# ounben/fishnet

Hardware: AMD Instinct MI355X
Metric: NNUE evals/sec (node) at 1/2/4/8 MI355X + FT gather HBM GB/s as % of peak (higher is better)
Workload: dtype int16/int8

## Files before the change

fishnet_amd/build.py:

```python
from __future__ import annotations

import os
import subprocess
import sys

HERE = os.path.dirname(os.path.abspath(__file__))
ROOT = os.path.dirname(HERE)
CSRC = os.path.join(HERE, "csrc")
LIBDIR = os.path.join(HERE, "lib")
LIB = os.path.join(LIBDIR, "libgpu_nnue.so")
FAULT_LIB = os.path.join(LIBDIR, "libgpu_nnue_fault.so")
FAULT_DEFINES = ("-DGN_FAULT_PLAN_BLOCK=1",)
ODD_LIB = os.path.join(LIBDIR, "libgpu_nnue_d5.so")
ODD_DEFINES = ("-DGN_SMALL_DEPTH=5",)
SOURCES = ["gpu_nnue.hip", "kernels.hip", "stream.hip"]
HEADERS = ["chess.h", "host_board.h", "nnue.h", "kernels.h", "sha256.h", "device_util.h", "archive.h"]
ARCH = "gfx950"


def source_hash(defines=()) -> str:
    import hashlib
    h = hashlib.sha256()
    deps = [os.path.join(CSRC, f) for f in SOURCES + HEADERS] + [os.path.join(ROOT, "include", "gpu_nnue.h")]
    for d in deps:
        h.update(os.path.basename(d).encode() + b"\0")
        with open(d, "rb") as f:
            h.update(f.read())
    h.update(" ".join([ARCH, *defines]).encode())
    return h.hexdigest()


def _stale(lib: str, defines=()) -> bool:
    stamp = lib + ".sha256"
    if not os.path.exists(lib) or not os.path.exists(stamp):
        return True
    with open(stamp) as f:
        return f.read().strip() != source_hash(defines)


def build(force: bool = False, verbose: bool = False, defines=(), out: str | None = None) -> str:
    lib = out or LIB
    if not force and not _stale(lib, defines):
        return lib
    os.makedirs(LIBDIR, exist_ok=True)
    objs = []
    for src in SOURCES:
        obj = os.path.join(LIBDIR, src.replace(".hip", f".{os.getpid()}.o"))
        cmd = ["hipcc", f"--offload-arch={ARCH}", "-O3", "-std=c++17", "-fPIC", "-fvisibility=hidden",
               "-Wall", "-Wno-unused-function", *defines, "-c", os.path.join(CSRC, src), "-o", obj]
        if verbose:
            print(" ".join(cmd), flush=True)
        subprocess.run(cmd, check=True)
        objs.append(obj)
    tmp = lib + f".tmp{os.getpid()}"
    cmd = ["hipcc", f"--offload-arch={ARCH}", "-shared", "-fPIC", "-o", tmp] + objs + ["-lpthread"]
    subprocess.run(cmd, check=True)
    os.replace(tmp, lib)
    with open(lib + ".sha256", "w") as f:
        f.write(source_hash(defines) + "\n")
    for o in objs:
        os.remove(o)
    return lib


def build_rev(rev: str, out: str, defines=()) -> str:
    import shutil
    import tempfile
    tmp = tempfile.mkdtemp(prefix="gn_rev_")
    try:
        arch = subprocess.run(["git", "-C", ROOT, "archive", rev, "fishnet_amd/csrc", "include"],
                              check=True, capture_output=True).stdout
        subprocess.run(["tar", "-x", "-C", tmp], input=arch, check=True)
        objs = []
        for src in SOURCES:
            obj = os.path.join(tmp, src.replace(".hip", ".o"))
            subprocess.run(["hipcc", f"--offload-arch={ARCH}", "-O3", "-std=c++17", "-fPIC", "-fvisibility=hidden",
                            "-w", *defines, "-c", os.path.join(tmp, "fishnet_amd", "csrc", src), "-o", obj],
                           check=True)
            objs.append(obj)
        lib = os.path.join(LIBDIR, out)
        subprocess.run(["hipcc", f"--offload-arch={ARCH}", "-shared", "-fPIC", "-o", lib] + objs + ["-lpthread"],
                       check=True)
        return lib
    finally:
        shutil.rmtree(tmp, ignore_errors=True)


def build_fault(force: bool = False, verbose: bool = False) -> str:
    return build(force=force, verbose=verbose, defines=FAULT_DEFINES, out=FAULT_LIB)


def build_odd(force: bool = False, verbose: bool = False) -> str:
    return build(force=force, verbose=verbose, defines=ODD_DEFINES, out=ODD_LIB)


DROPIN_NATIVE = os.path.join(LIBDIR, "dropin_native")


def build_dropin_native(force: bool = False) -> str:
# ... 22 lines not shown
```

fishnet_amd/csrc/device_util.h:

```cpp
#pragma once
#include <hip/hip_runtime.h>

#include "nnue.h"

namespace gn {

typedef unsigned short ushort8 __attribute__((ext_vector_type(8)));
typedef int int4v __attribute__((ext_vector_type(4)));

__device__ __forceinline__ int32_t wmul(int32_t a, int32_t b) { return (int32_t)((uint32_t)a * (uint32_t)b); }
__device__ __forceinline__ int32_t wadd(int32_t a, int32_t b) { return (int32_t)((uint32_t)a + (uint32_t)b); }
__device__ __forceinline__ int clampi(int v, int lo, int hi) { return v < lo ? lo : v > hi ? hi : v; }
__device__ __forceinline__ uint32_t ft_row(uint32_t idx) { return idx < FT_INPUTS ? idx : FT_INPUTS - 1; }

__device__ __forceinline__ void load_tables(Tables &dst, const Tables *src) {
  const uint4 *s = reinterpret_cast<const uint4 *>(src);
  uint4 *d = reinterpret_cast<uint4 *>(&dst);
  for (int i = threadIdx.x; i < (int)(sizeof(Tables) / 16); i += blockDim.x) d[i] = s[i];
  __syncthreads();
}

template <bool U>
__device__ __forceinline__ int uni(int x) {
  if constexpr (U) return __builtin_amdgcn_readfirstlane(x);
  else return x;
}

__device__ __forceinline__ ushort8 ldft(const uint8_t *__restrict__ ft, uint32_t off) {
  return *reinterpret_cast<const ushort8 *>(ft + off);
}
__device__ __forceinline__ uint32_t ldpd(const uint8_t *__restrict__ ft, uint32_t off) {
  return *reinterpret_cast<const uint32_t *>(ft + off);
}
__device__ __forceinline__ int4v ldps(const uint8_t *__restrict__ ft, uint32_t off) {
  return *reinterpret_cast<const int4v *>(ft + off);
}

__device__ __forceinline__ int wave_features(const gn_board &p, uint16_t *rows_w, uint16_t *rows_b, int lane) {
  const uint64_t occ = p.occ;
  const int c = popcnt(occ);
  const bool has = (occ >> lane) & 1;
  const int k = popcnt(occ & ((1ull << lane) - 1));
  uint64_t wlo, whi;
  piece_words(p, wlo, whi);
  const int pc = has && k < 32 ? piece_nibble(wlo, whi, k) : 0;
  const int pt = pc & 7;
  const uint64_t bad = __ballot(has && (pt < PAWN || pt > KING));
  const uint64_t wkb = __ballot(has && pc == make_piece(WHITE, KING));
  const uint64_t bkb = __ballot(has && pc == make_piece(BLACK, KING));
  if (c < 2 || c > 32 || bad || popcnt(wkb) != 1 || popcnt(bkb) != 1) return 0;
  if (has) {
    if (rows_w) rows_w[k] = (uint16_t)feature_index(WHITE, lane, pc, __builtin_ctzll(wkb));
    if (rows_b) rows_b[k] = (uint16_t)feature_index(BLACK, lane, pc, __builtin_ctzll(bkb));
  }
  return c;
}

__device__ __forceinline__ int lane_piece(const gn_board &p, int lane) {
  const uint64_t occ = p.occ;
  const bool has = (occ >> lane) & 1;
  const int k = popcnt(occ & ((1ull << lane) - 1));
  uint64_t wlo, whi;
  piece_words(p, wlo, whi);
  return has && k < 32 ? piece_nibble(wlo, whi, k) : 0;
}

__device__ __forceinline__ int wave_features_excl(const gn_board &p, uint16_t *rows_w, uint16_t *rows_b, int lane,
                                                  uint64_t excl) {
  const uint64_t occ = p.occ;
  const int c = popcnt(occ);
  const bool has = (occ >> lane) & 1;
  const int pc = lane_piece(p, lane);
  const int pt = pc & 7;
  const uint64_t bad = __ballot(has && (pt < PAWN || pt > KING));
  const uint64_t wkb = __ballot(has && pc == make_piece(WHITE, KING));
  const uint64_t bkb = __ballot(has && pc == make_piece(BLACK, KING));
  if (c < 2 || c > 32 || bad || popcnt(wkb) != 1 || popcnt(bkb) != 1) return 0;
  if (has && !((excl >> lane) & 1)) {
    const int k = popcnt(occ & ~excl & ((1ull << lane) - 1));
    rows_w[k] = (uint16_t)feature_index(WHITE, lane, pc, __builtin_ctzll(wkb));
    rows_b[k] = (uint16_t)feature_index(BLACK, lane, pc, __builtin_ctzll(bkb));
  }
  return c;
}

__device__ __forceinline__ void wave_features_king_move(const gn_board &p, int h, int kfrom, int kto, int rfrom,
                                                        int rto, uint16_t *rows, int lane) {
  const uint64_t occ = p.occ;
  const bool has = (occ >> lane) & 1;
  const int k = popcnt(occ & ((1ull << lane) - 1));
  uint64_t wlo, whi;
  piece_words(p, wlo, whi);
  int pc = has && k < 32 ? piece_nibble(wlo, whi, k) : 0;
  if (lane == kfrom || lane == rfrom) pc = 0;
  if (lane == rto) pc = make_piece(h, ROOK);
  if (lane == kto) pc = make_piece(h, KING);
  const uint64_t cocc = __ballot(pc != 0);
  if (pc) rows[popcnt(cocc & ((1ull << lane) - 1))] = (uint16_t)feature_index(h, lane, pc, kto);
}

typedef short short2v __attribute__((ext_vector_type(2)));
typedef unsigned short ushort2v __attribute__((ext_vector_type(2)));
__device__ __forceinline__ uint2 transform8(ushort8 lo, ushort8 hi) {
  uint32_t o[4];
  const short2v z = {0, 0}, m = {254, 254};
#pragma unroll
  for (int i = 0; i < 4; ++i) {
    short2v a = {(short)lo[2 * i], (short)lo[2 * i + 1]}, b = {(short)hi[2 * i], (short)hi[2 * i + 1]};
    a = __builtin_elementwise_min(__builtin_elementwise_max(a, z), m);
    b = __builtin_elementwise_min(__builtin_elementwise_max(b, z), m);
    ushort2v pr = __builtin_bit_cast(ushort2v, a) * __builtin_bit_cast(ushort2v, b);
    pr = pr >> (ushort2v){9, 9};
    o[i] = __builtin_bit_cast(uint32_t, pr);
  }
  return make_uint2(__builtin_amdgcn_perm(o[1], o[0], 0x06040200u), __builtin_amdgcn_perm(o[3], o[2], 0x06040200u));
}

template <int L1, class Valid, class Emit>
__device__ __forceinline__ void layer_stack_wave(const NetDevice &net, const uint8_t *xt, uint8_t (*in1)[32],
                                                 int32_t *fwd, const int32_t (*psq)[2], int b, int lane,
                                                 Valid &&valid, Emit &&emit) {
  constexpr int XS = L1 + 16, KS = L1 / 64, BATCH = KS % 6 == 0 ? 6 : KS % 4 == 0 ? 4 : KS;
  static_assert(KS % BATCH == 0, "k-steps per batch");
  const int row = lane & 15, kg = lane >> 4;
  const int4v zero = {0, 0, 0, 0};
  const int4v wl = *reinterpret_cast<const int4v *>(net.w1 + ((size_t)b * 32 + row) * 32 + (kg & 1) * 16);
  const int4v wh = *reinterpret_cast<const int4v *>(net.w1 + ((size_t)b * 32 + 16 + row) * 32 + (kg & 1) * 16);
  const int32_t bias0 = net.b0[b * 16 + row];
  const int32_t b1l = net.b1[b * 32 + row], b1h = net.b1[b * 32 + 16 + row];
  const int32_t w2l = net.w2[b * 32 + row], w2h = net.w2[b * 32 + 16 + row];
  const int32_t b2v = net.b2[b];
  constexpr bool FRAG = L1 > 128;
  const int8_t *wb = FRAG ? net.w0f + ((size_t)b * KS * 64 + lane) * 16 : net.w0 + ((size_t)b * 16 + row) * L1 + kg * 16;
  const uint8_t *xa = xt + row * XS + kg * 16;
  int4v acc = zero;
#pragma unroll 1
  for (int k0 = 0; k0 < KS; k0 += BATCH) {
    int4v w[BATCH], a[BATCH];
#pragma unroll
    for (int j = 0; j < BATCH; ++j) w[j] = *reinterpret_cast<const int4v *>(wb + (FRAG ? 1024 : 64) * (k0 + j));
#pragma unroll
    for (int j = 0; j < BATCH; ++j) a[j] = *reinterpret_cast<const int4v *>(xa + 64 * (k0 + j));
#pragma unroll
    for (int j = 0; j < BATCH; ++j) acc = __builtin_amdgcn_mfma_i32_16x16x64_i8(a[j], w[j], acc, 0, 0, 0);
  }
#pragma unroll
  for (int i = 0; i < 4; ++i) {
    const int pos = 4 * kg + i;
    const int32_t v = wadd(acc[i], bias0);
    if (row < 15) {
      const long long s2 = ((long long)v * v) >> 19;
      in1[pos][row] = (uint8_t)(s2 < 127 ? s2 : 127);
      in1[pos][15 + row] = (uint8_t)clampi(v >> 6, 0, 127);
    } else {
      fwd[pos] = wmul(v, 600 * 16) / (127 * 64);
      in1[pos][30] = 0;
      in1[pos][31] = 0;
    }
  }
  __builtin_amdgcn_fence(__ATOMIC_RELEASE, "wavefront");
  __builtin_amdgcn_wave_barrier();
  __builtin_amdgcn_fence(__ATOMIC_ACQUIRE, "wavefront");
  const int4v a1 = kg < 2 ? *reinterpret_cast<const int4v *>(&in1[row][kg * 16]) : zero;
  const int4v cl = __builtin_amdgcn_mfma_i32_16x16x64_i8(a1, wl, zero, 0, 0, 0);
  const int4v ch = __builtin_amdgcn_mfma_i32_16x16x64_i8(a1, wh, zero, 0, 0, 0);
  int32_t part[4];
#pragma unroll
  for (int i = 0; i < 4; ++i) {
    const int32_t l = clampi(wadd(cl[i], b1l) >> 6, 0, 127), hh = clampi(wadd(ch[i], b1h) >> 6, 0, 127);
    part[i] = w2l * l + w2h * hh;
  }
#pragma unroll
  for (int off = 8; off; off >>= 1)
#pragma unroll
    for (int i = 0; i < 4; ++i) part[i] = wadd(part[i], __shfl_xor(part[i], off, 16));
  if (row == 0) {
#pragma unroll
    for (int i = 0; i < 4; ++i) {
      const int pos = 4 * kg + i;
      if (valid(pos, b)) {
        const int32_t positional = wadd(wadd(b2v, part[i]), fwd[pos]);
        const int32_t psqt = (int32_t)((uint32_t)psq[pos][0] - (uint32_t)psq[pos][1]) / 2;
        emit(pos, make_int2(psqt / 16, positional / 16));
      }
    }
  }
}

__device__ __forceinline__ int king_move_row(const gn_board &pb, int h, int kf, int kt, int rf, int rt, int lane,
                                             int &pos, int *piece = nullptr) {
  const uint64_t occ = pb.occ;
  const bool has = (occ >> lane) & 1;
  const int k = popcnt(occ & ((1ull << lane) - 1));
  uint64_t wlo, whi;
  piece_words(pb, wlo, whi);
  int pc = has && k < 32 ? piece_nibble(wlo, whi, k) : 0;
  if (lane == kf || lane == rf) pc = 0;
  if (lane == rt) pc = make_piece(h, ROOK);
  if (lane == kt) pc = make_piece(h, KING);
  const uint64_t cocc = __ballot(pc != 0);
  pos = popcnt(cocc & ((1ull << lane) - 1));
  if (piece) *piece = pc;
  return pc ? feature_index(h, lane, pc, kt) : -1;
}

__device__ __forceinline__ int king_move_row_pc(int pc, int h, int kf, int kt, int rf, int rt, int lane, int &pos,
                                                int &piece) {
  if (lane == kf || lane == rf) pc = 0;
  if (lane == rt) pc = make_piece(h, ROOK);
  if (lane == kt) pc = make_piece(h, KING);
  const uint64_t cocc = __ballot(pc != 0);
  pos = popcnt(cocc & ((1ull << lane) - 1));
  piece = pc;
  return pc ? feature_index(h, lane, pc, kt) : -1;
}

__device__ __forceinline__ int32_t wave_sum(int32_t v) {
#pragma unroll
  for (int off = 32; off; off >>= 1) v = wadd(v, __shfl_xor(v, off));
  return v;
}

template <class Op>
__device__ __forceinline__ uint32_t dpp_scan(uint32_t x, Op op) {
  x = op(x, (uint32_t)__builtin_amdgcn_update_dpp(0, (int)x, 0x111, 0xf, 0xf, true));
  x = op(x, (uint32_t)__builtin_amdgcn_update_dpp(0, (int)x, 0x112, 0xf, 0xf, true));
  x = op(x, (uint32_t)__builtin_amdgcn_update_dpp(0, (int)x, 0x114, 0xf, 0xf, true));
  x = op(x, (uint32_t)__builtin_amdgcn_update_dpp(0, (int)x, 0x118, 0xf, 0xf, true));
  x = op(x, (uint32_t)__builtin_amdgcn_update_dpp(0, (int)x, 0x142, 0xa, 0xf, false));
  x = op(x, (uint32_t)__builtin_amdgcn_update_dpp(0, (int)x, 0x143, 0xc, 0xf, false));
  return x;
}
__device__ __forceinline__ uint32_t scan_add(uint32_t x) {
  return dpp_scan(x, [](uint32_t a, uint32_t b) { return a + b; });
}
__device__ __forceinline__ uint32_t scan_or(uint32_t x) {
  return dpp_scan(x, [](uint32_t a, uint32_t b) { return a | b; });
}
__device__ __forceinline__ uint32_t or8(uint32_t x) {
  x |= (uint32_t)__builtin_amdgcn_update_dpp(0, (int)x, 0xb1, 0xf, 0xf, false);
  x |= (uint32_t)__builtin_amdgcn_update_dpp(0, (int)x, 0x4e, 0xf, 0xf, false);
  x |= (uint32_t)__builtin_amdgcn_update_dpp(0, (int)x, 0x141, 0xf, 0xf, false);
  return x;
}
__device__ __forceinline__ int32_t wave_sum_dpp(int32_t v) {
  return __builtin_amdgcn_readlane((int)scan_add((uint32_t)v), 63);
}

__device__ __forceinline__ void stage_fc1(int4v *w1s, const NetDevice &net) {
  for (int i = threadIdx.x; i < 8 * 32 * 2; i += blockDim.x) w1s[i] = reinterpret_cast<const int4v *>(net.w1)[i];
}
template <int NPART>
__device__ __forceinline__ void slice_sums(const int32_t *__restrict__ part, uint64_t npos, uint64_t q, int4v (&sums)[4]) {
#pragma unroll
  for (int r = 0; r < 4; ++r) {
    sums[r] = *reinterpret_cast<const int4v *>(part + q * 16 + 4 * r);
#pragma unroll
    for (int t = 1; t < NPART; ++t) {
      const int4v c = *reinterpret_cast<const int4v *>(part + ((uint64_t)t * npos + q) * 16 + 4 * r);
#pragma unroll
      for (int k = 0; k < 4; ++k) sums[r][k] = wadd(sums[r][k], c[k]);
    }
  }
}
__device__ __forceinline__ int2 slice_finish_from(const NetDevice &net, const int4v *w1s, const int4v (&sums)[4],
                                                  int2 info) {
  const int b = info.y & 7;
  int32_t v[16];
#pragma unroll
  for (int r = 0; r < 16; ++r) v[r] = wadd(sums[r >> 2][r & 3], net.b0[b * 16 + r]);
  uint32_t x[8] = {0, 0, 0, 0, 0, 0, 0, 0};
#pragma unroll
  for (int r = 0; r < 15; ++r) {
    const uint32_t u = v[r] < 0 ? 0u - (uint32_t)v[r] : (uint32_t)v[r], m = u < 8160u ? u : 8160u;
    const uint32_t a = (m * m) >> 19, c = (uint32_t)clampi(v[r] >> 6, 0, 127);
    x[r >> 2] |= a << (8 * (r & 3));
    x[(15 + r) >> 2] |= c << (8 * ((15 + r) & 3));
  }
  const int32_t fwd = wmul(v[15], 600 * 16) / (127 * 64);
  int32_t sum = 0;
#pragma unroll 4
  for (int o = 0; o < 32; ++o) {
    const int4v wa = w1s[(b * 32 + o) * 2], wb = w1s[(b * 32 + o) * 2 + 1];
    int32_t acc = 0;
#pragma unroll
    for (int d = 0; d < 4; ++d) acc = __builtin_amdgcn_sdot4((int)x[d], wa[d], acc, false);
#pragma unroll
    for (int d = 0; d < 4; ++d) acc = __builtin_amdgcn_sdot4((int)x[4 + d], wb[d], acc, false);
    const int32_t l = clampi(wadd(acc, net.b1[b * 32 + o]) >> 6, 0, 127);
    sum = wadd(sum, (int32_t)net.w2[b * 32 + o] * l);
  }
  const int32_t positional = wadd(wadd(net.b2[b], sum), fwd);
  return make_int2(info.x / 16, positional / 16);
}
template <int NPART>
__device__ __forceinline__ int2 slice_finish_one(const NetDevice &net, const int4v *w1s, const int32_t *__restrict__ part,
                                                 uint64_t npos, uint64_t q, int2 info) {
  int4v sums[4];
  slice_sums<NPART>(part, npos, q, sums);
  return slice_finish_from(net, w1s, sums, info);
}

}
```

fishnet_amd/csrc/gpu_nnue.hip:

```cpp
#include <stdarg.h>
#include <stdio.h>
#include <string.h>

#include <algorithm>
#include <atomic>
#include <chrono>
#include <condition_variable>
#include <memory>
#include <mutex>
#include <string>
#include <thread>
#include <vector>

#include "archive.h"
#include "host_board.h"
#include "kernels.h"
#include "sha256.h"

using namespace gn;

static thread_local std::string g_err;

static int fail(int code, const char *fmt, ...) {
  char buf[512];
// ... 159 lines not shown
  int mode = -1;
  uint64_t gen = 0;
  hipGraph_t graph = nullptr;
  hipGraphExec_t exec = nullptr;
  hipEvent_t done = nullptr;
  bool busy = false;
  gn_board *h_in = nullptr;
  gn_eval *h_out = nullptr;
  DevBuf<gn_board> all;
  DevBuf<gn_eval> rec;
  gn_board *in = nullptr, *r1 = nullptr, *r2 = nullptr;
  gn_eval *out = nullptr, *e1 = nullptr, *e2 = nullptr;
  DevBuf<uint64_t> off0, off1;
  DevBuf<uint16_t> m1, m2;
  DevBuf<int32_t> sv1, sv2;
  EvalBufs eb;
  ~FastBatch() {
    if (done) (void)hipEventDestroy(done);
    if (exec) (void)hipGraphExecDestroy(exec);
    if (graph) (void)hipGraphDestroy(graph);
    if (h_in) (void)hipHostFree(h_in);
    if (h_out) (void)hipHostFree(h_out);
    all.release(), rec.release();
    off0.release(), off1.release(), m1.release(), m2.release(), sv1.release(), sv2.release();
    eb.release();
  }
};

struct ExpSet {
  DevBuf<uint64_t> counts, offsets;
  DevBuf<uint32_t> owner;
  DevBuf<Board> unpacked;
  DevBuf<uint16_t> moves_tmp;
  const uint16_t *child_moves = nullptr;
  DevBuf<int2> pinfo;
  DevBuf<int2> p_osm, p_obg;
  DevBuf<uint8_t> p_nsm, p_nbg;
  EvalBufs eb;
  DevBuf<gn_board> children;
  int chain_k = 1;
  int slices = 1;
  bool planned = false;
  uint64_t etot = 0;
  void *scan_tmp = nullptr, *sort_tmp = nullptr;
  size_t scan_bytes = 0, sort_bytes = 0;
  hipEvent_t scored = nullptr;
  DevBuf<uint32_t> perr;
  DevBuf<unsigned long long> pstat;
  DevBuf<uint64_t> ent, eoff;
  DevBuf<TileDesc> tiles;
  DevBuf<uint32_t> btiles, border;
  void release() {
    perr.release(), pstat.release();
    ent.release(), eoff.release(), tiles.release(), btiles.release(), border.release();
    counts.release(), offsets.release(), owner.release(), unpacked.release(), moves_tmp.release();
    pinfo.release(), p_osm.release(), p_obg.release(), p_nsm.release(), p_nbg.release(), eb.release();
    children.release();
    if (scan_tmp) (void)hipFree(scan_tmp);
    if (sort_tmp) (void)hipFree(sort_tmp);
    scan_tmp = sort_tmp = nullptr, scan_bytes = sort_bytes = 0;
    if (scored) (void)hipEventDestroy(scored);
    scored = nullptr;
  }
};

struct Dev {
  int id = 0;
  hipStream_t stream = nullptr;
  void *net_mem[2] = {nullptr, nullptr};
  NetDevice net[2] = {};
  bool has[2] = {false, false};
  Tables *tables = nullptr;
  ExpSet cur, alt;
  DevBuf<gn_board> io_boards, frontier;
  DevBuf<gn_eval> io_out, io_out2;
  DevBuf<uint32_t> off32;
  DevBuf<uint16_t> moves;
  DevBuf<ChildDelta> deltas;
  DevBuf<uint64_t> kkeys, kkeys2;
  DevBuf<uint32_t> kidx, kperm;
  DevBuf<unsigned long long> sum;
  DevBuf<uint8_t> nslot;
  DevBuf<int32_t> part;
  bool part_locked = false;
  DevBuf<uint64_t> ebound;
  DevBuf<uint32_t> pool;
  DevBuf<uint16_t> bkeys, bkeys2;
  DevBuf<uint32_t> bidx;
  hipEvent_t done = nullptr;
  hipStream_t done_on = nullptr;
  float plan_ms = 0, stream_ms = 0, finish_ms = 0;
  struct ScoreLevel {
    DevBuf<uint64_t> sel, pos, counts, offsets;
    DevBuf<uint32_t> idx, owner;
    DevBuf<gn_board> boards, children;
    DevBuf<uint16_t> moves;
    DevBuf<gn_eval> ce;
    DevBuf<int32_t> sv;
    void release() {
      sel.release(), pos.release(), counts.release(), offsets.release(), idx.release(), owner.release();
      boards.release(), children.release(), moves.release(), ce.release(), sv.release();
    }
  } lv[2];
  hipStream_t copy = nullptr;
  hipEvent_t cev[2] = {nullptr, nullptr};
  DevBuf<gn_eval> po2[2], co2[2];
  DevBuf<gn_child> cc2[2];
  DevBuf<gn_line> ln2[2];
  hipEvent_t rev[2] = {nullptr, nullptr};
  DevBuf<uint16_t> mv2[2];
  DevBuf<gn_board> roots, rboards, par;
  DevBuf<uint64_t> moff;
  DevBuf<uint16_t> codes, smoves;
  DevBuf<int32_t> rstatus;
  DevBuf<uint32_t> gidx;
  double t_upload = 0, t_replay = 0, t_compute = 0, t_download = 0, t_tail = 0, t_rank = 0;
  std::unique_ptr<FastBatch> fast[6][3][2];
  std::condition_variable fast_cv;
  hipStream_t front = nullptr;
  hipEvent_t ev_streamed = nullptr, ev_planned = nullptr;
  std::mutex mu;
};

static void swap_sets(Dev &d) { std::swap(d.cur, d.alt); }

static hipError_t seq_begin(Dev &d, hipStream_t s) {
  if (d.done_on && d.done_on != s) return hipStreamWaitEvent(s, d.done, 0);
  return hipSuccess;
}
static hipError_t seq_end(Dev &d, hipStream_t s) {
  hipError_t e = hipEventRecord(d.done, s);
  if (e == hipSuccess) d.done_on = s;
  return e;
}
static int check_plan(Dev &d, hipStream_t s) {
  if (!d.cur.planned || !d.cur.perr.p) return GN_OK;
  uint32_t e = 0;
  HIP_TRY(hipMemcpyAsync(&e, d.cur.perr.p, sizeof(e), hipMemcpyDeviceToHost, s));
  HIP_TRY(hipStreamSynchronize(s));
  if (e) return fail(GN_E_HIP, "planned expansion failed on the device (error bits 0x%x)", e);
  return GN_OK;
}

struct SeqGuard {
  Dev &d;
  hipStream_t s;
  hipError_t e;
  bool ended = false;
  SeqGuard(Dev &d_, hipStream_t s_) : d(d_), s(s_) { e = seq_begin(d, s); }
  hipError_t finish() {
    ended = true;
    hipError_t r = seq_end(d, s);
    return r == hipSuccess ? hipStreamSynchronize(s) : r;
  }
  ~SeqGuard() {
    if (!ended) (void)seq_end(d, s);
  }
};

#ifndef GN_MAX_LEADERS
#define GN_MAX_LEADERS 1
#endif
constexpr int MAX_LEADERS = GN_MAX_LEADERS;
struct BatchReq {
  const gn_board *boards;
  size_t n;
// ... 23 lines not shown
  bool incremental = true;
  int swizzle = 9;
  int king_sort = 1;
  int chain = 81;
  bool king_cache = true;
  int stream_slices = 3;
  int64_t chunk_parents = 0;
  int l1[2] = {0, 0};
  uint32_t hash[2] = {0, 0};
  double t_parse = 0, t_total = 0;
};

enum { BIG = 0, SMALL = 1 };

static gn_eval_params default_params() {
  gn_eval_params P;
  P.small_net_threshold = 962;
  P.psqt_weight = 125;
  P.positional_weight = 131;
  P.reeval_threshold = 236;
  P.complexity_div_small = 18000;
  P.complexity_div_big = 18000;
  P.material_pawn_small = 535;
  P.material_pawn_big = 535;
  P.material_base = 77777;
  P.rule50_div = 212;
  P.value_clamp = 31506;
  const int32_t pv[5] = {208, 781, 825, 1276, 2538};
  memcpy(P.piece_value, pv, sizeof(pv));
  const double wa[4] = {-37.45051876, 121.19101539, -132.78783573, 420.70576692};
  memcpy(P.wdl_a, wa, sizeof(wa));
  P.wdl_material_min = 17;
  P.wdl_material_max = 78;
  P.wdl_material_anchor = 58;
  const int32_t ww[5] = {1, 3, 3, 5, 9};
  memcpy(P.wdl_piece_weight, ww, sizeof(ww));
  return P;
}

static size_t align256(size_t x) { return (x + 255) & ~(size_t)255; }

static int upload_net(Dev &d, int which, const HostNet &h) {
  const size_t RS = ft_row_stride((uint32_t)h.L1);
  size_t off[10], o = 0;
  const int carry = h.L1 == 128 ? 0 : CARRY_SLOTS;
  std::vector<int32_t> psqt((size_t)PSQT_BUCKETS * FT_ROWS);
  for (size_t r = 0; r < (size_t)FT_ROWS; ++r)
    for (int b = 0; b < PSQT_BUCKETS; ++b)
      memcpy(&psqt[(size_t)b * FT_ROWS + r], h.ft.data() + r * RS + 2 * (size_t)h.L1 + 4 * b, 4);
  const int KS = h.L1 / 64;
  std::vector<int8_t> w0f(h.w0.size());
  for (int b = 0; b < LAYER_STACKS; ++b)
    for (int ks = 0; ks < KS; ++ks)
      for (int ln = 0; ln < 64; ++ln)
        memcpy(&w0f[(((size_t)b * KS + ks) * 64 + ln) * 16],
               &h.w0[((size_t)b * 16 + (ln & 15)) * h.L1 + 64 * (size_t)ks + 16 * (ln >> 4)], 16);
  const size_t sz[10] = {((size_t)FT_ROWS + 4 * (size_t)carry + 128 * (size_t)carry + (carry ? 1 : 0)) * RS, h.bias.size() * 2, h.w0.size(), h.b0.size() * 4,
                         h.w1.size(), h.b1.size() * 4, h.w2.size(), h.b2.size() * 4, psqt.size() * 4, w0f.size()};
  const void *src[10] = {h.ft.data(), h.bias.data(), h.w0.data(), h.b0.data(),
                         h.w1.data(), h.b1.data(), h.w2.data(), h.b2.data(), psqt.data(), w0f.data()};
  for (int i = 0; i < 10; ++i) off[i] = o, o += align256(sz[i]);
  uint8_t *m = nullptr;
  if (hipMalloc(&m, o) != hipSuccess) return fail(GN_E_NOMEM, "device allocation of %zu bytes failed", o);
  d.net_mem[which] = m;
  for (int i = 0; i < 10; ++i)
    HIP_TRY(hipMemcpy(m + off[i], src[i], i == 0 ? (size_t)FT_ROWS * RS : sz[i], hipMemcpyHostToDevice));
  if (carry) HIP_TRY(hipMemset(m + off[0] + (size_t)FT_ROWS * RS, 0, 4 * (size_t)carry * RS));
  if (carry) HIP_TRY(hipMemset(m + off[0] + (size_t)ZERO_ROW * RS, 0, RS));
  NetDevice &n = d.net[which];
  n.L1 = h.L1;
  n.row_stride = (uint32_t)RS;
  n.carry_slots = carry;
  n.kc_slots = carry;
  n.ft = m + off[0];
  n.bias = reinterpret_cast<const int16_t *>(m + off[1]);
  n.w0 = reinterpret_cast<const int8_t *>(m + off[2]);
  n.b0 = reinterpret_cast<const int32_t *>(m + off[3]);
  n.w1 = reinterpret_cast<const int8_t *>(m + off[4]);
  n.b1 = reinterpret_cast<const int32_t *>(m + off[5]);
  n.w2 = reinterpret_cast<const int8_t *>(m + off[6]);
  n.b2 = reinterpret_cast<const int32_t *>(m + off[7]);
  n.psqt = reinterpret_cast<const int32_t *>(m + off[8]);
  n.w0f = reinterpret_cast<const int8_t *>(m + off[9]);
  d.has[which] = true;
  return GN_OK;
}

static void destroy(gn_ctx *ctx) {
  if (!ctx) return;
  for (auto &dp : ctx->devs) {
    Dev &d = *dp;
    (void)hipSetDevice(d.id);
    if (d.stream) (void)hipStreamSynchronize(d.stream);
    for (void *m : d.net_mem)
      if (m) (void)hipFree(m);
    if (d.tables) (void)hipFree(d.tables);
    d.cur.release(), d.alt.release();
    d.io_boards.release(), d.frontier.release(), d.io_out.release(), d.io_out2.release();
    d.off32.release(), d.moves.release(), d.sum.release(), d.deltas.release();
    d.part.release();
    if (d.front) (void)hipStreamSynchronize(d.front), (void)hipStreamDestroy(d.front);
    if (d.ev_streamed) (void)hipEventDestroy(d.ev_streamed);
    if (d.ev_planned) (void)hipEventDestroy(d.ev_planned);
    d.kkeys.release(), d.kkeys2.release(), d.kidx.release(), d.kperm.release();
    d.nslot.release();
    d.ebound.release(), d.pool.release();
    d.bkeys.release(), d.bkeys2.release(), d.bidx.release();
    d.lv[0].release(), d.lv[1].release();
    for (auto &row : d.fast)
      for (auto &pair : row)
        for (auto &f : pair) f.reset();
    for (int i = 0; i < 2; ++i) {
      d.po2[i].release(), d.co2[i].release(), d.cc2[i].release(), d.mv2[i].release(), d.ln2[i].release();
      if (d.rev[i]) (void)hipEventDestroy(d.rev[i]);
      if (d.cev[i]) (void)hipEventDestroy(d.cev[i]);
    }
    d.roots.release(), d.rboards.release(), d.par.release(), d.moff.release(), d.codes.release();
    d.smoves.release(), d.rstatus.release(), d.gidx.release();
    if (d.copy) (void)hipStreamSynchronize(d.copy), (void)hipStreamDestroy(d.copy);
    if (d.done) (void)hipEventDestroy(d.done);
    if (d.stream) (void)hipStreamDestroy(d.stream);
  }
  delete ctx;
}

static int create(const uint8_t *big, size_t big_len, const uint8_t *small, size_t small_len, const int *devices,
                  int n_devices, gn_ctx **out) {
  if (!out) return fail(GN_E_INVALID, "out is NULL");
  *out = nullptr;
  if (!big && !small) return fail(GN_E_INVALID, "no network given");
  HostNet hn[2];
  if (big) {
    int rc = parse_net(big, big_len, hn[BIG]);
    if (rc) return rc;
  }
  if (small) {
    int rc = parse_net(small, small_len, hn[SMALL]);
    if (rc) return rc;
  }
  int count = 0;
  if (hipGetDeviceCount(&count) != hipSuccess || count <= 0) return fail(GN_E_NODEVICE, "no HIP device visible");
  std::vector<int> ids;
  if (devices && n_devices > 0) ids.assign(devices, devices + n_devices);
  else ids.push_back(0);
  std::unique_ptr<gn_ctx, void (*)(gn_ctx *)> ctx(new gn_ctx(), destroy);
  ctx->P = default_params();
  for (int w = 0; w < 2; ++w) ctx->l1[w] = hn[w].L1, ctx->hash[w] = hn[w].hash;
  for (int id : ids) {
    if (id < 0 || id >= count) return fail(GN_E_NODEVICE, "device %d out of range (%d visible)", id, count);
    hipDeviceProp_t prop;
    HIP_TRY(hipGetDeviceProperties(&prop, id));
    if (!strstr(prop.gcnArchName, "gfx950"))
      return fail(GN_E_NODEVICE, "device %d is %s; libgpu_nnue is built for gfx950 only", id, prop.gcnArchName);
    ctx->devs.emplace_back(new Dev());
    Dev &d = *ctx->devs.back();
    d.id = id;
    HIP_TRY(hipSetDevice(id));
    HIP_TRY(hipStreamCreateWithFlags(&d.stream, hipStreamNonBlocking));
    HIP_TRY(hipEventCreateWithFlags(&d.done, hipEventDisableTiming));
    HIP_TRY(hipStreamCreateWithFlags(&d.copy, hipStreamNonBlocking));
#ifdef GN_AB_FRONT_PRIORITY
    {
      int least = 0, greatest = 0;
      HIP_TRY(hipDeviceGetStreamPriorityRange(&least, &greatest));
      HIP_TRY(hipStreamCreateWithPriority(&d.front, hipStreamNonBlocking, greatest));
    }
// ... 56 lines not shown
  DevBuf<int2> &osm = B.osm, &obg = B.obg;
  DevBuf<uint8_t> &nsm = B.nsm, &nbg = B.nbg;
  if (mode != GN_MODE_BIG) HIP_TRY(osm.ensure(n));
  if (mode != GN_MODE_SMALL) HIP_TRY(obg.ensure(n));
  if (mode == GN_MODE_FULL) {
    HIP_TRY(nsm.ensure(n));
    HIP_TRY(nbg.ensure(n));
  }
  auto mark = [&](int k) -> hipError_t { return ev ? hipEventRecord(ev[k], s) : hipSuccess; };
  const gn_eval_params &P = ctx->P;
  HIP_TRY(mark(0));
  const uint32_t *perm = nullptr;
  constexpr size_t KING_SORT_MIN = 1024;
  if (sort && (ctx->king_sort == 2 || (ctx->king_sort == 1 && n >= KING_SORT_MIN))) {
    if (n > 0x7FFFFFFFull) return fail(GN_E_INVALID, "king sort supports < 2^31 positions per call");
    HIP_TRY(d.kkeys.ensure(n));
    HIP_TRY(d.kkeys2.ensure(n));
    HIP_TRY(d.kidx.ensure(n));
    HIP_TRY(d.kperm.ensure(n));
    HIP_TRY(king_sort(b, n, d.kkeys.p, d.kidx.p, d.kkeys2.p, d.kperm.p, mode != GN_MODE_SMALL, d.cur.sort_tmp,
                      d.cur.sort_bytes, s));
    perm = d.kperm.p;
  }
  const int swz = (ctx->swizzle >> 1) & 1;
  HIP_TRY(mark(1));
  if (mode == GN_MODE_FULL && d.net[SMALL].L1 != 128) {
    HIP_TRY(launch_classify(b, n, P, nsm.p, nbg.p, s));
    HIP_TRY(launch_eval_net(d.net[SMALL], b, nsm.p, n, osm.p, perm, swz, s, nullptr));
    HIP_TRY(launch_reeval(osm.p, nsm.p, n, P, nbg.p, s));
  } else if (mode != GN_MODE_BIG)
    HIP_TRY(launch_eval_net(d.net[SMALL], b, nullptr, n, osm.p, perm, swz, s, mode == GN_MODE_SMALL ? rows_out : nullptr,
                            mode == GN_MODE_FULL ? &P : nullptr, nsm.p, nbg.p));
  HIP_TRY(mark(2));
  if (mode != GN_MODE_SMALL)
    HIP_TRY(launch_eval_net(d.net[BIG], b, mode == GN_MODE_FULL ? nbg.p : nullptr, n, obg.p, perm, swz, s,
                            rows_out));
  HIP_TRY(mark(3));
  HIP_TRY(launch_finalize(b, n, mode, osm.p, obg.p, nsm.p, nbg.p, P, d.tables, out, s, score, counts));
  HIP_TRY(mark(4));
  return GN_OK;
}

static Dev *slot(gn_ctx *ctx, int s) {
  if (!ctx || s < 0 || s >= (int)ctx->devs.size()) return nullptr;
  return ctx->devs[s].get();
}

template <class F>
static void parallel_for(size_t n, size_t grain, F &&f) {
  unsigned hw = std::max(1u, std::min(16u, std::thread::hardware_concurrency()));
  size_t chunks = std::min<size_t>(hw, (n + grain - 1) / std::max<size_t>(grain, 1));
  if (chunks <= 1) {
    f(0, n);
    return;
  }
  std::vector<std::thread> th;
  size_t per = (n + chunks - 1) / chunks;
  for (size_t c = 0; c < chunks; ++c) {
    size_t lo = c * per, hi = std::min(n, lo + per);
    if (lo < hi) th.emplace_back([=, &f] { f(lo, hi); });
  }
  for (auto &t : th) t.join();
}

static int chain_len(const gn_ctx *ctx, Dev &d, size_t n) {
  if (!ctx->incremental || (ctx->chain >= -1 && ctx->chain <= 1) || !d.has[BIG] || !d.net[BIG].carry_slots)
    return 1;
  if (ctx->chain < 0) return -ctx->chain;
  size_t k = (size_t)ctx->chain;
  if ((n + k - 1) / k < 2048) k = std::max<size_t>(2, std::min(k, n / 2048));
  return (int)k;
}

static bool plan_path(const gn_ctx *ctx, const Dev &d, int mode) {
  return mode != GN_MODE_SMALL && ctx->incremental && d.has[BIG] &&
         (d.net[BIG].L1 == 3072 || d.net[BIG].L1 == 1024);
}

static int finalize_all(gn_ctx *ctx, Dev &d, const gn_board *parents, const gn_board *children, int mode,
                        gn_eval *parent_out, gn_eval *child_out, size_t n, size_t total, hipStream_t s,
                        bool score_parents, bool sliced = false) {
  const gn_eval_params &P = ctx->P;
  const ExpSet &x = d.cur;
  const SlicedOut sc = {&d.net[BIG], d.part.p, x.pinfo.p, (uint64_t)(n + total), (uint64_t)n},
                  sp = {&d.net[BIG], d.part.p, x.pinfo.p, (uint64_t)(n + total), 0};
  const bool fast = x.child_moves != nullptr;
  HIP_TRY(launch_finalize(children, total, mode, x.eb.osm.p, x.eb.obg.p, x.eb.nsm.p, x.eb.nbg.p, P, d.tables, child_out,
                          s, 0, nullptr, fast ? x.owner.p : nullptr, fast ? x.child_moves : nullptr,
                          fast ? x.unpacked.p : nullptr, sliced ? &sc : nullptr));
  if (parent_out)
    HIP_TRY(launch_finalize(parents, n, mode, x.p_osm.p, x.p_obg.p, x.p_nsm.p, x.p_nbg.p, P, d.tables, parent_out, s,
                            score_parents ? 1 : 0, x.counts.p, nullptr, nullptr, nullptr, sliced ? &sp : nullptr));
  return GN_OK;
}

static hipError_t count_children(Dev &d, const gn_board *parents, size_t n, hipStream_t s, size_t *total) {
  ExpSet &x = d.cur;
  hipError_t e;
  if ((e = x.counts.ensure(n + 1)) != hipSuccess || (e = x.offsets.ensure(n + 1)) != hipSuccess) return e;
  if ((e = hipMemsetAsync(x.counts.p + n, 0, sizeof(uint64_t), s)) != hipSuccess) return e;
  if ((e = launch_count_children(parents, n, d.tables, x.counts.p, s)) != hipSuccess) return e;
  if ((e = exclusive_scan_u64(x.counts.p, x.offsets.p, n + 1, x.scan_tmp, x.scan_bytes, s)) != hipSuccess) return e;
  uint64_t t = 0;
  if ((e = hipMemcpyAsync(&t, x.offsets.p + n, sizeof(t), hipMemcpyDeviceToHost, s)) != hipSuccess) return e;
  if ((e = hipStreamSynchronize(s)) != hipSuccess) return e;
  *total = (size_t)t;
  return hipSuccess;
}

struct GenOpts {
  hipEvent_t *ev = nullptr;
  unsigned long long *rows = nullptr;
  bool deltas = false;
  int chain_k = 1;
  bool plan = false;
  bool skip_internal = false;
  bool trusted = false;
  size_t limit = SIZE_MAX;
};
static int generate_children(Dev &d, const gn_board *parents, size_t n, gn_board *children_or_null, uint16_t *moves,
                             size_t *total, hipStream_t s, const GenOpts &o = {}) {
  ExpSet &x = d.cur;
  x.chain_k = o.deltas ? o.chain_k : 1;
  x.planned = o.deltas && o.plan;
  if (x.planned) {
    HIP_TRY(hipMemsetAsync(x.perr.p, 0, sizeof(uint32_t), s));
    HIP_TRY(hipMemsetAsync(x.pstat.p, 0, sizeof(unsigned long long), s));
  }
  if (x.chain_k > 1) HIP_TRY(d.nslot.ensure(n));
  HIP_TRY(x.counts.ensure(n + 1));
  HIP_TRY(x.offsets.ensure(n + 1));
  HIP_TRY(hipMemsetAsync(x.counts.p + n, 0, sizeof(uint64_t), s));
  if (x.planned) {
    HIP_TRY(d.ebound.ensure(n + 1));
    HIP_TRY(x.eoff.ensure(n + 1));
    HIP_TRY(hipMemsetAsync(d.ebound.p + n, 0, sizeof(uint64_t), s));
  }
  HIP_TRY(launch_count_children(parents, n, d.tables, x.counts.p, s, x.planned ? d.ebound.p : nullptr, o.trusted));
  HIP_TRY(exclusive_scan_u64(x.counts.p, x.offsets.p, n + 1, x.scan_tmp, x.scan_bytes, s));
  if (x.planned) HIP_TRY(exclusive_scan_u64(d.ebound.p, x.eoff.p, n + 1, x.scan_tmp, x.scan_bytes, s));
  if (o.ev) HIP_TRY(hipEventRecord(o.ev[0], s));
  uint64_t t = 0;
  HIP_TRY(hipMemcpyAsync(&t, x.offsets.p + n, sizeof(t), hipMemcpyDeviceToHost, s));
  if (x.planned) HIP_TRY(hipMemcpyAsync(&x.etot, x.eoff.p + n, sizeof(uint64_t), hipMemcpyDeviceToHost, s));
  HIP_TRY(hipStreamSynchronize(s));
  *total = (size_t)t;
  if (t > o.limit) return fail(GN_E_CAPACITY, "%zu children exceed capacity %zu", (size_t)t, o.limit);
  if (o.ev) HIP_TRY(hipEventRecord(o.ev[1], s));
  gn_board *children = children_or_null;
  const bool skip_boards = !children_or_null && x.planned && o.skip_internal;
  if (!children && !skip_boards) {
    HIP_TRY(x.children.ensure(std::max<size_t>(t, 1)));
    children = x.children.p;
  }
  if (o.deltas) HIP_TRY(d.deltas.ensure(std::max<size_t>(t, 1)));
  HIP_TRY(x.owner.ensure(std::max<size_t>(t, 1)));
  HIP_TRY(x.unpacked.ensure(std::max<size_t>(n, 1)));
  if (!moves) {
    HIP_TRY(x.moves_tmp.ensure(std::max<size_t>(t, 1)));
    moves = x.moves_tmp.p;
  }
  x.child_moves = moves;
  if (t) {
    HIP_TRY(launch_write_children(parents, n, d.tables, x.offsets.p, 0, t, children, moves, x.owner.p,
                                  o.deltas ? d.deltas.p : nullptr, x.chain_k > 1 ? d.nslot.p : nullptr, x.chain_k,
                                  o.rows, s, x.unpacked.p, o.trusted));
  }
  if (o.ev) HIP_TRY(hipEventRecord(o.ev[2], s));
  return GN_OK;
}

static GenOpts gen_opts(const gn_ctx *ctx, Dev &d, size_t n, int mode, size_t limit) {
  GenOpts g;
  g.deltas = ctx->incremental, g.chain_k = chain_len(ctx, d, n), g.plan = plan_path(ctx, d, mode);
  g.skip_internal = mode == GN_MODE_BIG, g.limit = limit;
  return g;
}

constexpr int EXP_FRONT = 1, EXP_BACK = 2;
struct EvalOpts {
  hipEvent_t *ev = nullptr;
  unsigned long long *rows = nullptr;
  bool score_parents = true;
  int phases = EXP_FRONT | EXP_BACK;
  hipEvent_t streamed = nullptr;
};
static int expand_evaluate(gn_ctx *ctx, Dev &d, const gn_board *parents, size_t n, const gn_board *children,
                           size_t total, int mode, gn_eval *parent_out, gn_eval *child_out, hipStream_t s,
                           const EvalOpts &o = {}) {
  if (mode < GN_MODE_FULL || mode > GN_MODE_SMALL) return fail(GN_E_INVALID, "bad mode %d", mode);
  if ((mode != GN_MODE_SMALL && !d.has[BIG]) || (mode != GN_MODE_BIG && !d.has[SMALL]))
    return fail(GN_E_NONET, "mode %d needs a network that is not loaded", mode);
  ExpSet &x = d.cur;
  hipEvent_t *const ev = o.ev;
  const int phases = o.phases;
  if (!ctx->incremental) {
    if (!(phases & EXP_BACK)) return GN_OK;
    if (total) {
      int rc = evaluate_on(ctx, d, children, total, mode, child_out, s, nullptr, nullptr, 0);
      if (rc) return rc;
    }
    return parent_out ? evaluate_on(ctx, d, parents, n, mode, parent_out, s, nullptr, nullptr, o.score_parents ? 1 : 0,
                                    x.counts.p)
                      : GN_OK;
  }
  auto mark = [&](int k) -> hipError_t { return ev ? hipEventRecord(ev[k], s) : hipSuccess; };
  const gn_eval_params &P = ctx->P;
  const uint64_t *off = x.offsets.p;
  const ChildDelta *dl = d.deltas.p;
  const bool f = mode == GN_MODE_FULL;
  const size_t K = (size_t)std::max(1, x.chain_k), nblk = (n + K - 1) / K;
  const bool ordered = ctx->king_sort && nblk > 1;
  auto plan_args = [&] {
    PlanStreamArgs a;
    a.parents = parents, a.n = n, a.offsets = off, a.deltas = dl;
    a.need_parent = f ? x.p_nbg.p : nullptr, a.need_child = f ? x.eb.nbg.p : nullptr;
    a.out_parent = x.p_obg.p, a.out_child = x.eb.obg.p;
    a.next_slot = x.chain_k > 1 ? d.nslot.p : nullptr, a.chain_k = x.chain_k, a.kc = ctx->king_cache ? 1 : 0;
    a.eoff = x.eoff.p, a.ent = x.ent.p, a.tiles = x.tiles.p, a.btiles = x.btiles.p;
    a.pool = d.pool.p, a.err = x.perr.p, a.rows_out = o.rows, a.pads_out = x.pstat.p;
    a.slices = x.slices, a.npos = n + total;
    if (x.slices > 1) a.part = d.part.p, a.pinfo = x.pinfo.p;
    return a;
  };
  if (phases & EXP_FRONT) {
    const size_t nt = std::max<size_t>(total, 1);
    if (mode != GN_MODE_BIG) {
      HIP_TRY(x.eb.osm.ensure(nt));
      HIP_TRY(x.p_osm.ensure(n));
    }
    if (mode != GN_MODE_SMALL) {
      HIP_TRY(x.eb.obg.ensure(nt));
      HIP_TRY(x.p_obg.ensure(n));
    }
    if (f) {
      HIP_TRY(x.eb.nsm.ensure(nt));
      HIP_TRY(x.eb.nbg.ensure(nt));
      HIP_TRY(x.p_nsm.ensure(n));
      HIP_TRY(x.p_nbg.ensure(n));
      HIP_TRY(launch_classify(parents, n, P, x.p_nsm.p, x.p_nbg.p, s));
      HIP_TRY(launch_classify(children, total, P, x.eb.nsm.p, x.eb.nbg.p, s));
    }
    HIP_TRY(mark(0));
    if (mode != GN_MODE_BIG) {
      HIP_TRY(launch_expand_net(d.net[SMALL], parents, n, off, children, dl, f ? x.p_nsm.p : nullptr,
                                f ? x.eb.nsm.p : nullptr, x.p_osm.p, x.eb.osm.p, ctx->swizzle & 1, s));
      if (f) {
        HIP_TRY(launch_reeval(x.p_osm.p, x.p_nsm.p, n, P, x.p_nbg.p, s));
        HIP_TRY(launch_reeval(x.eb.osm.p, x.eb.nsm.p, total, P, x.eb.nbg.p, s));
      }
    }
    HIP_TRY(mark(1));
    x.slices = 1;
    if (mode != GN_MODE_SMALL && x.planned) {
      HIP_TRY(x.ent.ensure(x.etot + (size_t)ENT_SPARE * (nblk + 1)));
      HIP_TRY(x.tiles.ensure((n + total) / 16 + (K + 2) * nblk + 2));
      HIP_TRY(x.btiles.ensure(nblk + 1));
      HIP_TRY(d.pool.ensure(88));
      if (d.net[BIG].L1 == 3072 && ctx->stream_slices == 3) {
        const size_t need = (size_t)GN_PART_SLICES * 16 * (n + total);
        bool ok = d.part_locked ? d.part.cap >= need : d.part.ensure(need) == hipSuccess;
        ok = ok && x.pinfo.ensure(n + total) == hipSuccess;
        if (ok) x.slices = 3;
        else {
          (void)hipGetLastError();
          if (!d.part_locked) d.part.release();
          x.pinfo.release();
        }
      }
      if (ordered) {
        HIP_TRY(d.bkeys.ensure(nblk));
        HIP_TRY(d.bkeys2.ensure(nblk));
        HIP_TRY(d.bidx.ensure(nblk));
        HIP_TRY(x.border.ensure(nblk));
        HIP_TRY(block_order(parents, n, (uint32_t)K, (uint32_t)nblk, d.bkeys.p, d.bidx.p, d.bkeys2.p, x.border.p,
                            x.sort_tmp, x.sort_bytes, s));
      }
      PlanStreamArgs a = plan_args();
      a.mid = ev ? ev[4] : nullptr;
      HIP_TRY(launch_plan_stream(d.net[BIG], a, PLAN_PHASE, s));
    }
  }
  if (!(phases & EXP_BACK)) return GN_OK;
  bool fused = false;
  if (mode != GN_MODE_SMALL) {
    if (x.planned) {
      HIP_TRY(hipMemsetAsync(d.pool.p, 0, 88 * sizeof(uint32_t), s));
#ifndef GN_AB_FINISH_SEPARATE
      fused = x.slices > 1;
#endif
      if (ev && (phases & EXP_FRONT) == 0) HIP_TRY(hipEventRecord(ev[7], s));
      PlanStreamArgs a = plan_args();
      a.swz = (ctx->swizzle >> 2) & 1 ? 1 : (ctx->swizzle >> 3) & 1 ? 2 : 0;
      a.order = ordered ? x.border.p : nullptr;
      a.fin = ev ? ev[6] : nullptr, a.streamed = o.streamed, a.finish = !fused;
      HIP_TRY(launch_plan_stream(d.net[BIG], a, STREAM_PHASE, s));
    } else {
      HIP_TRY(launch_expand_net(d.net[BIG], parents, n, off, children, dl, f ? x.p_nbg.p : nullptr,
                                f ? x.eb.nbg.p : nullptr, x.p_obg.p, x.eb.obg.p, ctx->swizzle & 1, s));
    }
  }
  HIP_TRY(mark(2));
  int rc = finalize_all(ctx, d, parents, children, mode, parent_out, child_out, n, total, s, o.score_parents, fused);
  if (rc) return rc;
  HIP_TRY(mark(3));
  return GN_OK;
}

struct Replies {
  const gn_eval *rec;
  const uint16_t *moves;
};
static int resolve_scores(gn_ctx *ctx, Dev &d, const gn_board *boards, size_t n, int mode, gn_eval *out,
                          int32_t *sv_out, hipStream_t s, int depth = 2, const Replies *replies = nullptr) {
  if (!n || depth <= 0 || !out) return GN_OK;
  Dev::ScoreLevel &L = d.lv[2 - depth];
  HIP_TRY(L.sel.ensure(n + 1));
  HIP_TRY(L.pos.ensure(n + 1));
  HIP_TRY(launch_score_select(out, n, L.sel.p, s));
  HIP_TRY(exclusive_scan_u64(L.sel.p, L.pos.p, n + 1, d.cur.scan_tmp, d.cur.scan_bytes, s));
  uint64_t m = 0;
  HIP_TRY(hipMemcpyAsync(&m, L.pos.p + n, sizeof(m), hipMemcpyDeviceToHost, s));
  HIP_TRY(hipStreamSynchronize(s));
  if (!m) return GN_OK;
  HIP_TRY(L.idx.ensure(m));
  HIP_TRY(L.boards.ensure(m));
  HIP_TRY(L.counts.ensure(m + 1));
  HIP_TRY(L.offsets.ensure(m + 1));
  HIP_TRY(launch_score_gather(boards, L.sel.p, L.pos.p, n, replies ? nullptr : d.tables, L.idx.p, L.boards.p, s));
  if (replies) {
    uint64_t t = 0;
    HIP_TRY(launch_score_replies(L.idx.p, m, d.cur.offsets.p, L.counts.p, L.offsets.p, d.cur.scan_tmp,
                                 d.cur.scan_bytes, &t, s));
    HIP_TRY(L.moves.ensure(std::max<uint64_t>(t, 1)));
    HIP_TRY(L.children.ensure(std::max<uint64_t>(t, 1)));
    HIP_TRY(L.ce.ensure(std::max<uint64_t>(t, 1)));
    HIP_TRY(L.sv.ensure(std::max<uint64_t>(t, 1)));
    HIP_TRY(launch_score_replies_fill(L.idx.p, m, d.cur.offsets.p, L.offsets.p, replies->rec, replies->moves,
                                      d.cur.unpacked.p, d.tables, L.ce.p, L.children.p, L.moves.p, s));
    int rc = resolve_scores(ctx, d, L.children.p, t, mode, L.ce.p, L.sv.p, s, depth - 1);
    if (rc) return rc;
    HIP_TRY(launch_score_reduce(L.boards.p, m, L.idx.p, L.offsets.p, L.moves.p, L.ce.p, L.sv.p, ctx->P, out, sv_out,
                                s));
// ... 348 lines not shown
      auto it = std::lower_bound(starts.begin(), starts.end(), x);
      x = it == starts.end() ? m : *it;
    }
    if (x > c.back() && x < m) c.push_back(x);
  }
  c.push_back(m);
  return c;
}

static int count_shard(Dev &d, const gn_board *d_par, size_t m, std::vector<uint64_t> &off) {
  size_t total = 0;
  HIP_TRY(count_children(d, d_par, m, d.stream, &total));
  off.resize(m + 1);
  HIP_TRY(hipMemcpy(off.data(), d.cur.offsets.p, (m + 1) * sizeof(uint64_t), hipMemcpyDeviceToHost));
  return GN_OK;
}

struct ExpStep {
  const gn_board *parents = nullptr;
  size_t n = 0;
  gn_eval *parent_out = nullptr, *child_out = nullptr;
  uint16_t *moves = nullptr;
  size_t cap = SIZE_MAX;
  hipEvent_t *ev = nullptr;
  unsigned long long *rows = nullptr;
};
static bool pipelined(const gn_ctx *ctx, const Dev &d, int mode, size_t count) {
  return ctx->pipeline && plan_path(ctx, d, mode) && ctx->incremental && count > 1;
}
template <class Step, class Done>
static int run_expansions(gn_ctx *ctx, Dev &d, int mode, size_t count, size_t largest, Step &&step, Done &&done) {
  if (!count) return GN_OK;
  const hipStream_t s = d.stream;
  const bool pipe = pipelined(ctx, d, mode, count);
  const hipStream_t F = pipe ? d.front : s;
  struct Guard {
    Dev &d;
    bool pipe, ok = false;
    ~Guard() {
      d.part_locked = false;
      if (pipe && !ok) (void)hipStreamSynchronize(d.front);
    }
  } guard{d, pipe};
  struct Queued {
    ExpStep st;
    size_t total = 0;
    gn_eval *po = nullptr, *co = nullptr;
  } q[2];
  auto front = [&](size_t i) -> int {
    Queued &x = q[i & 1];
    x = Queued();
    int rc = step(i, x.st);
    if (rc) return rc;
    const ExpStep &st = x.st;
    if (st.ev) HIP_TRY(hipEventRecord(st.ev[0], F));
    GenOpts g = gen_opts(ctx, d, st.n, mode, st.cap);
    g.ev = st.ev ? st.ev + 1 : nullptr, g.rows = g.plan ? nullptr : st.rows;
    if ((rc = generate_children(d, st.parents, st.n, nullptr, st.moves, &x.total, F, g)) != GN_OK) return rc;
    if (!st.parent_out) HIP_TRY(d.io_out.ensure(st.n));
    if (!st.child_out) HIP_TRY(d.io_out2.ensure(std::max<size_t>(x.total, 1)));
    x.po = st.parent_out ? st.parent_out : d.io_out.p, x.co = st.child_out ? st.child_out : d.io_out2.p;
    if (!pipe) return GN_OK;
    EvalOpts e;
    e.ev = st.ev ? st.ev + 4 : nullptr, e.rows = st.rows ? st.rows + 1 : nullptr, e.phases = EXP_FRONT;
    rc = expand_evaluate(ctx, d, st.parents, st.n, d.cur.children.p, x.total, mode, nullptr, nullptr, F, e);
    if (rc) return rc;
    HIP_TRY(hipEventRecord(d.ev_planned, F));
    return GN_OK;
  };
  auto next_front = [&](size_t i) -> int {
    swap_sets(d);
    int rc = GN_OK;
    if (hipStreamWaitEvent(F, ctx->pipeline == 2 ? d.cur.scored : d.ev_streamed, 0) != hipSuccess)
      rc = fail(GN_E_HIP, "hipStreamWaitEvent failed");
    if (!rc) rc = front(i);
    swap_sets(d);
    return rc;
  };
  if (pipe) {
    HIP_TRY(hipEventRecord(d.ev_streamed, s));
    HIP_TRY(hipStreamWaitEvent(F, d.ev_streamed, 0));
    if (largest) {
      if (d.has[BIG] && d.net[BIG].L1 == 3072 && ctx->stream_slices == 3 &&
          d.part.ensure((size_t)GN_PART_SLICES * 16 * largest) != hipSuccess)
        (void)hipGetLastError();
      d.part_locked = true;
    }
  }
  int rc = front(0);
  d.part_locked = pipe;
  for (size_t i = 0; i < count && rc == GN_OK; ++i) {
    const Queued &x = q[i & 1];
    const bool more = i + 1 < count;
    EvalOpts e;
    e.ev = x.st.ev ? x.st.ev + 4 : nullptr, e.rows = x.st.rows ? x.st.rows + 1 : nullptr;
    if (pipe) {
      HIP_TRY(hipStreamWaitEvent(s, d.ev_planned, 0));
      e.phases = EXP_BACK, e.streamed = d.ev_streamed;
    }
    rc = expand_evaluate(ctx, d, x.st.parents, x.st.n, d.cur.children.p, x.total, mode, x.po, x.co, s, e);
    if (rc || (pipe && more && (rc = next_front(i + 1)) != GN_OK)) return rc;
    const Replies rp{x.co, d.cur.child_moves};
    if ((rc = resolve_scores(ctx, d, x.st.parents, x.st.n, mode, x.po, nullptr, s, 2, &rp)) != GN_OK) return rc;
    if (pipe) HIP_TRY(hipEventRecord(d.cur.scored, s));
    rc = done(i, x.total);
    if (rc || !more) break;
    if (pipe) swap_sets(d);
    else rc = front(i + 1);
  }
  guard.ok = rc == GN_OK;
  return rc;
}

static int expand_pipelined(gn_ctx *ctx, Dev &d, const gn_board *d_par, size_t m, int mode,
                            const std::vector<uint64_t> &off, const std::vector<size_t> &chunks, gn_eval *parent_out,
                            uint16_t *child_moves, gn_child *child_out, int n_lines = 0, gn_line *lines = nullptr) {
  hipStream_t s = d.stream;
  size_t maxp = 1, maxc = 1;
  for (size_t c = 0; c + 1 < chunks.size(); ++c)
    maxp = std::max(maxp, chunks[c + 1] - chunks[c]),
    maxc = std::max<size_t>(maxc, off[chunks[c + 1]] - off[chunks[c]]);
  for (int k = 0; k < 2; ++k) {
    HIP_TRY(d.po2[k].ensure(maxp));
    HIP_TRY(d.co2[k].ensure(maxc));
    if (n_lines) HIP_TRY(d.ln2[k].ensure(maxp * (size_t)n_lines));
    else HIP_TRY(d.cc2[k].ensure(maxc));
    HIP_TRY(d.mv2[k].ensure(maxc));
  }
  int drc[2] = {GN_OK, GN_OK};
  std::string derr[2];
  double dms[2] = {0, 0};
  std::thread drain[2];
  struct Joiner {
    std::thread *t;
    ~Joiner() {
      for (int i = 0; i < 2; ++i)
        if (t[i].joinable()) t[i].join();
    }
  } joiner{drain};
  auto join = [&](int k) -> int {
    if (drain[k].joinable()) drain[k].join();
    d.t_download += dms[k], dms[k] = 0;
    if (!drc[k]) return GN_OK;
    const int r = drc[k];
    drc[k] = GN_OK;
    g_err = derr[k];
    return r;
  };
  auto drain_chunk = [&](int k, size_t pa, size_t mp, size_t t, uint64_t cb) {
    drain[k] = std::thread([&, k, pa, mp, t, cb] {
      const auto t1 = Clock::now();
      hipError_t e = hipSetDevice(d.id);
      if (e == hipSuccess) e = hipStreamWaitEvent(d.copy, d.cev[k], 0);
      if (e == hipSuccess && n_lines)
        e = hipMemcpyAsync(lines + pa * (size_t)n_lines, d.ln2[k].p, mp * (size_t)n_lines * sizeof(gn_line),
                           hipMemcpyDeviceToHost, d.copy);
      if (e == hipSuccess && t && !n_lines)
        e = hipMemcpyAsync(child_out + cb, d.cc2[k].p, t * sizeof(gn_child), hipMemcpyDeviceToHost, d.copy);
      if (e == hipSuccess && t && !n_lines)
        e = hipMemcpyAsync(child_moves + cb, d.mv2[k].p, t * sizeof(uint16_t), hipMemcpyDeviceToHost, d.copy);
      if (e == hipSuccess && parent_out)
        e = hipMemcpyAsync(parent_out + pa, d.po2[k].p, mp * sizeof(gn_eval), hipMemcpyDeviceToHost, d.copy);
      if (e == hipSuccess) e = hipStreamSynchronize(d.copy);
      if (e != hipSuccess) drc[k] = GN_E_HIP, derr[k] = std::string("result download failed: ") + hipGetErrorString(e);
      dms[k] = ms_since(t1);
    });
  };
// ... 1144 lines not shown
  }
}

int gn_get_option(const gn_ctx *ctx, int option, int64_t *value) {
  if (!ctx || !value) return fail(GN_E_INVALID, "NULL argument");
  switch (option) {
  case GN_OPT_INCREMENTAL_CHILDREN:
    *value = ctx->incremental;
    return GN_OK;
  case GN_OPT_XCD_SWIZZLE:
    *value = ctx->swizzle;
    return GN_OK;
  case GN_OPT_KING_SORT:
    *value = ctx->king_sort;
    return GN_OK;
  case GN_OPT_KING_CACHE:
    *value = ctx->king_cache;
    return GN_OK;
  case GN_OPT_CHAIN:
    *value = ctx->chain;
    return GN_OK;
  case GN_OPT_STREAM_SLICES:
    *value = ctx->stream_slices;
    return GN_OK;
  case GN_OPT_CHUNK_PARENTS:
    *value = ctx->chunk_parents;
    return GN_OK;
  case GN_OPT_COALESCE:
    *value = ctx->coalesce;
    return GN_OK;
  case GN_OPT_FAST_BATCH:
    *value = ctx->fast_batch;
    return GN_OK;
  case GN_OPT_EXPAND_PIPELINE:
    *value = ctx->pipeline;
    return GN_OK;
  case GN_STAT_FAST_BATCHES:
    *value = (int64_t)ctx->fast_runs.load();
    return GN_OK;
  case GN_STAT_FAST_FALLBACKS:
    *value = (int64_t)ctx->fast_fallbacks.load();
    return GN_OK;
  case GN_STAT_BATCH_LAUNCHES:
  case GN_STAT_BATCH_CALLS: {
    auto &C = const_cast<gn_ctx *>(ctx)->co;
    std::lock_guard<std::mutex> lk(C.mu);
    *value = (int64_t)(option == GN_STAT_BATCH_LAUNCHES ? C.launches : C.calls);
    return GN_OK;
  }
  case GN_STAT_PLAN_NS:
  case GN_STAT_STREAM_NS:
  case GN_STAT_FINISH_NS: {
    float m = 0;
    for (auto &dp : ctx->devs)
      m = std::max(m, option == GN_STAT_PLAN_NS     ? dp->plan_ms
                      : option == GN_STAT_STREAM_NS ? dp->stream_ms
                                                    : dp->finish_ms);
    *value = (int64_t)((double)m * 1e6);
    return GN_OK;
  }
  case GN_STAT_HOST_PARSE_NS:
  case GN_STAT_HOST_TOTAL_NS:
    *value = (int64_t)((option == GN_STAT_HOST_PARSE_NS ? ctx->t_parse : ctx->t_total) * 1e6);
    return GN_OK;
  case GN_STAT_HOST_UPLOAD_NS:
  case GN_STAT_HOST_REPLAY_NS:
  case GN_STAT_HOST_COMPUTE_NS:
  case GN_STAT_HOST_DOWNLOAD_NS:
  case GN_STAT_RANK_NS:
  case GN_STAT_HOST_TAIL_NS: {
    double m = 0;
    for (auto &dp : ctx->devs) {
      const Dev &d = *dp;
      m = std::max(m, option == GN_STAT_HOST_UPLOAD_NS    ? d.t_upload
                      : option == GN_STAT_HOST_REPLAY_NS  ? d.t_replay
                      : option == GN_STAT_HOST_COMPUTE_NS ? d.t_compute
                      : option == GN_STAT_HOST_DOWNLOAD_NS ? d.t_download
                      : option == GN_STAT_RANK_NS          ? d.t_rank
                                                           : d.t_tail);
    }
    *value = (int64_t)(m * 1e6);
    return GN_OK;
  }
  case GN_STAT_SCRATCH_PADS: {
    int64_t sum = 0;
    for (auto &dp : ctx->devs) {
      Dev &d = *dp;
      std::lock_guard<std::mutex> lk(d.mu);
      if (!d.cur.pstat.p) continue;
      HIP_TRY(hipSetDevice(d.id));
      if (d.done_on) HIP_TRY(hipEventSynchronize(d.done));
      unsigned long long v = 0;
      HIP_TRY(hipMemcpy(&v, d.cur.pstat.p, sizeof(v), hipMemcpyDeviceToHost));
      sum += (int64_t)v;
    }
    *value = sum;
    return GN_OK;
  }
  default:
    return fail(GN_E_INVALID, "unknown option %d", option);
  }
}

int gn_expand_and_evaluate(gn_ctx *ctx, const char *const *parent_fens, size_t n, int mode, gn_eval *parent_out,
                           uint32_t *child_offsets, uint16_t *child_moves, gn_child *child_out, size_t cap) {
  if (!slot(ctx, 0)) return fail(GN_E_INVALID, "bad context");
  if (n && (!parent_fens || !child_offsets)) return fail(GN_E_INVALID, "NULL argument");
  if (!n) {
    if (child_offsets) child_offsets[0] = 0;
    return GN_OK;
  }
  try {
    const auto T0 = Clock::now();
    reset_host_stats(ctx);
    std::vector<gn_board> boards(n);
    int rc = gn_pack_fens(parent_fens, n, boards.data(), nullptr);
    if (rc) return rc;
    ctx->t_parse = ms_since(T0);
    rc = expand_boards_host(ctx, boards.data(), n, mode, parent_out, child_offsets, child_moves, child_out, cap);
    ctx->t_total = ms_since(T0);
    return rc;
  } catch (const std::bad_alloc &) {
    return fail(GN_E_NOMEM, "host allocation failed");
  } catch (...) {
    return fail(GN_E_INVALID, "unexpected exception");
  }
}

int gn_perft(gn_ctx *ctx, const char *fen, int depth, uint64_t *nodes) {
  Dev *d = slot(ctx, 0);
  if (!d || !fen || !nodes) return fail(GN_E_INVALID, "bad argument");
  Board B;
  if (!parse_fen(fen, B)) return fail(GN_E_INVALID, "bad FEN");
  if (depth <= 0) {
    *nodes = 1;
    return GN_OK;
  }
  std::lock_guard<std::mutex> lk(d->mu);
  HIP_TRY(hipSetDevice(d->id));
  hipStream_t s = d->stream;
  SeqGuard sg(*d, s);
  HIP_TRY(sg.e);
  gn_board root;
  pack(B, root);
  HIP_TRY(d->frontier.ensure(1));
  HIP_TRY(hipMemcpyAsync(d->frontier.p, &root, sizeof(root), hipMemcpyHostToDevice, s));
  size_t n = 1;
  for (int level = 1; level < depth; ++level) {
    size_t total = 0;
    int rc = generate_children(*d, d->frontier.p, n, nullptr, nullptr, &total, s);
    if (rc) return rc;
    std::swap(d->frontier, d->cur.children);
    n = total;
    if (!n) break;
  }
  unsigned long long sum = 0;
  if (n) {
    HIP_TRY(d->sum.ensure(1));
    HIP_TRY(hipMemsetAsync(d->sum.p, 0, sizeof(unsigned long long), s));
    HIP_TRY(launch_count_sum(d->frontier.p, n, d->tables, d->sum.p, s));
    HIP_TRY(hipMemcpyAsync(&sum, d->sum.p, sizeof(sum), hipMemcpyDeviceToHost, s));
  }
  HIP_TRY(hipStreamSynchronize(s));
  *nodes = sum;
  return GN_OK;
}
// ... 3 lines not shown
```

fishnet_amd/csrc/kernels.h:

```cpp
#pragma once
#include <hip/hip_runtime.h>
#include <stddef.h>
#include <stdint.h>

#include "nnue.h"

#ifndef GN_RING
#define GN_RING 4
#endif
#ifndef GN_SLICE_RING
#define GN_SLICE_RING 4
#endif
#ifndef GN_SCR_GAP
#define GN_SCR_GAP (GN_RING > GN_SLICE_RING ? GN_RING : GN_SLICE_RING)
#endif
#ifndef GN_FRONT_WG
#define GN_FRONT_WG 128
#endif
static_assert(GN_FRONT_WG == 64 || GN_FRONT_WG == 128 || GN_FRONT_WG == 256, "front workgroups of 1, 2 or 4 waves");

constexpr unsigned ENT_SPARE = 32;

#ifdef GN_PART_INPLACE
#define GN_PART_SLICES 1
#else
#define GN_PART_SLICES 3
#endif

namespace gn {

hipError_t launch_eval_net(const NetDevice &net, const gn_board *boards, const uint8_t *need, size_t n,
                           int2 *out, const uint32_t *perm, int swz, hipStream_t s,
                           unsigned long long *rows_out = nullptr, const gn_eval_params *cls = nullptr,
                           uint8_t *need_small = nullptr, uint8_t *need_big = nullptr);
hipError_t launch_checksum(const void *p, size_t bytes, unsigned long long *out, hipStream_t s);
hipError_t block_order(const gn_board *parents, size_t n, uint32_t K, uint32_t nblk, uint16_t *keys, uint32_t *idx,
                       uint16_t *keys_out, uint32_t *order, void *&temp, size_t &temp_bytes, hipStream_t s);
hipError_t king_sort(const gn_board *boards, size_t n, uint64_t *keys, uint32_t *idx, uint64_t *keys_out,
                     uint32_t *perm, bool placement, void *&temp, size_t &temp_bytes, hipStream_t s);
hipError_t launch_expand_net(const NetDevice &net, const gn_board *parents, size_t n, const uint64_t *offsets,
                             const gn_board *children, const ChildDelta *deltas, const uint8_t *need_parent,
                             const uint8_t *need_child, int2 *out_parent, int2 *out_child, int swz, hipStream_t s);
struct TileDesc {
  uint32_t e_end[2];
  uint32_t p_first;
  uint32_t first;
  uint8_t meta[16];
  int32_t psq[16][2];
  int16_t adj[16];
};
static_assert(sizeof(TileDesc) == 192, "TileDesc is 192 bytes");
constexpr int PLAN_PHASE = 1, STREAM_PHASE = 2;
struct PlanStreamArgs {
  const gn_board *parents = nullptr;
  size_t n = 0;
  const uint64_t *offsets = nullptr;
  const ChildDelta *deltas = nullptr;
  const uint8_t *need_parent = nullptr, *need_child = nullptr;
  int2 *out_parent = nullptr, *out_child = nullptr;
  const uint8_t *next_slot = nullptr;
  int chain_k = 1;
  int kc = 0;
  const uint64_t *eoff = nullptr;
  uint64_t *ent = nullptr;
  TileDesc *tiles = nullptr;
  uint32_t *btiles = nullptr;
  uint32_t *pool = nullptr;
  uint32_t *err = nullptr;
  unsigned long long *rows_out = nullptr;
  unsigned long long *pads_out = nullptr;
  const uint32_t *order = nullptr;
  int slices = 1;
  int32_t *part = nullptr;
  size_t npos = 0;
  int2 *pinfo = nullptr;
  bool finish = true;
  int swz = 0;
  hipEvent_t mid = nullptr;
  hipEvent_t fin = nullptr, streamed = nullptr;
};
hipError_t launch_plan_stream(const NetDevice &net, const PlanStreamArgs &a, int phases, hipStream_t s);
hipError_t launch_classify(const gn_board *boards, size_t n, const gn_eval_params &P, uint8_t *need_small,
                           uint8_t *need_big, hipStream_t s);
hipError_t launch_reeval(const int2 *out_small, const uint8_t *need_small, size_t n, const gn_eval_params &P,
                         uint8_t *need_big, hipStream_t s);
struct SlicedOut {
  const NetDevice *net;
  const int32_t *part;
  const int2 *pinfo;
  uint64_t npos, qoff;
};
hipError_t launch_finalize(const gn_board *boards, size_t n, int mode, const int2 *out_small,
                           const int2 *out_big, const uint8_t *need_small, const uint8_t *need_big,
                           const gn_eval_params &P, const Tables *tables, gn_eval *out, hipStream_t s,
                           int score, const uint64_t *counts = nullptr, const uint32_t *owner = nullptr,
                           const uint16_t *moves = nullptr, const Board *unpacked = nullptr,
                           const SlicedOut *sliced = nullptr);
hipError_t launch_score_select(const gn_eval *out, size_t n, uint64_t *sel, hipStream_t s);
hipError_t launch_score_gather(const gn_board *boards, const uint64_t *sel, const uint64_t *pos, size_t n,
                               const Tables *tables, uint32_t *idx, gn_board *sb, hipStream_t s);
hipError_t launch_score_replies(const uint32_t *idx, size_t m, const uint64_t *off, uint64_t *counts,
                                uint64_t *coff, void *&temp, size_t &temp_bytes, uint64_t *total_host, hipStream_t s);
hipError_t launch_score_replies_fill(const uint32_t *idx, size_t m, const uint64_t *off, const uint64_t *coff,
                                     const gn_eval *rec, const uint16_t *moves, const Board *unpacked,
                                     const Tables *tables, gn_eval *ce, gn_board *cb, uint16_t *cm, hipStream_t s);
hipError_t launch_score_reduce(const gn_board *sb, size_t m, const uint32_t *idx, const uint64_t *off,
                               const uint16_t *moves, const gn_eval *ce, const int32_t *csv, const gn_eval_params &P,
                               gn_eval *out, int32_t *sv, hipStream_t s);
hipError_t launch_score_reduce2(const gn_board *sb1, size_t m1, const uint64_t *off1, const uint16_t *moves2,
                                const gn_eval *ce2, const int32_t *csv2, gn_eval *out1, int32_t *sv1,
                                const gn_board *sb0, size_t m0, const uint64_t *off0, const uint16_t *moves1,
                                const gn_eval_params &P, gn_eval *out0, hipStream_t s);
hipError_t launch_reply_level(const gn_board *boards, size_t n, const Tables *tables, uint64_t *off, size_t cap,
                              gn_board *rb, uint16_t *rm, uint32_t *flag, int first, hipStream_t s);
hipError_t launch_count_children(const gn_board *boards, size_t n, const Tables *tables, uint64_t *counts,
                                 hipStream_t s, uint64_t *ebound = nullptr, bool trusted = false);
hipError_t launch_write_children(const gn_board *boards, size_t n, const Tables *tables, const uint64_t *offsets,
                                 size_t c0, size_t nc, gn_board *children, uint16_t *moves, uint32_t *owner,
                                 ChildDelta *deltas, uint8_t *next_slot, int chain_k, unsigned long long *rows,
                                 hipStream_t s, Board *unpacked = nullptr, bool trusted = false);
hipError_t launch_count_sum(const gn_board *boards, size_t n, const Tables *tables,
                            unsigned long long *total, hipStream_t s);
hipError_t launch_random_positions(uint64_t seed, size_t first, size_t n, int max_plies, const Tables *tables,
                                   gn_board *out, hipStream_t s);
hipError_t launch_random_games(uint64_t seed, size_t first_game, size_t n_games, int plies, const Tables *tables,
                               gn_board *out, hipStream_t s);
hipError_t launch_replay_games(const gn_board *roots, size_t ng, const uint64_t *moff, const uint16_t *codes,
                               const Tables *tables, gn_board *boards, uint16_t *smoves, int32_t *status, hipStream_t s);
hipError_t launch_gather_boards(const gn_board *src, const uint32_t *idx, size_t n, gn_board *dst, hipStream_t s);
hipError_t launch_pack_children(const gn_eval *in, size_t n, gn_child *out, hipStream_t s);
hipError_t launch_rank_children(const Board *unpacked, size_t n, const uint64_t *offsets, const uint16_t *moves,
                                const gn_eval *rec, const gn_eval_params &P, const Tables *tables, int K,
                                gn_line *lines, hipStream_t s);
hipError_t launch_rank_children(const gn_board *parents, size_t n, const uint32_t *offsets, const uint16_t *moves,
                                const gn_eval *rec, const gn_eval_params &P, const Tables *tables, int K,
                                gn_line *lines, hipStream_t s);
hipError_t launch_offsets_u32(const uint64_t *in, size_t n, uint32_t *out, hipStream_t s);
hipError_t exclusive_scan_u64(const uint64_t *counts, uint64_t *offsets, size_t n1, void *&temp,
                              size_t &temp_bytes, hipStream_t s);

}
```

fishnet_amd/csrc/kernels.hip:

```cpp
#include <stdio.h>
#include <stdlib.h>
#include <string.h>

#include <algorithm>

#include <hipcub/hipcub.hpp>

#include "device_util.h"
#include "kernels.h"

#ifndef GN_SMALL_DEPTH
#define GN_SMALL_DEPTH 4
#endif
#ifndef GN_SMALL_WPE
#define GN_SMALL_WPE 8
#endif


namespace gn {

constexpr int LS_SCRATCH = 16 * 16 * 4 + 16 * 32 + 16 * 4;

template <int L1, int NW, class Valid, class Emit>
__device__ __forceinline__ void layer_stack_tile(const NetDevice &net, const uint8_t *xt, uint8_t *ls,
// ... 575 lines not shown
        if (jt == 0) psq[sl][side] = (int32_t)ps;
      }
      __syncthreads();

      layer_stack_tile<L1, NW>(net, xt, scratch, psq, tl, bmask, [&](int pos, int bb) {
        return t0 + pos < total && valid[pos] && bkt[pos] == bb;
      }, [&](int pos, int2 val) {
        if (t0 + pos == 0) out_parent[p] = val;
        else out_child[off + t0 + pos - 1] = val;
      });
    }
  }
}

hipError_t launch_eval_net(const NetDevice &net, const gn_board *boards, const uint8_t *need, size_t n, int2 *out,
                           const uint32_t *perm, int swz, hipStream_t s, unsigned long long *rows_out,
                           const gn_eval_params *cls, uint8_t *need_small, uint8_t *need_big) {
  if (cls && (net.L1 != 128 || !need_small || !need_big)) return hipErrorInvalidValue;
  const gn_eval_params P = cls ? *cls : gn_eval_params{};
  if (!n) return hipSuccess;
  unsigned tn = 16;
#ifndef GN_TN_MIN
#define GN_TN_MIN (n <= 1024 ? 1u : 2u)
#endif
#ifndef GN_AB_TN16
  if (net.L1 != 128)
    while (tn > (GN_TN_MIN) && (n + tn - 1) / tn < 2048) tn >>= 1;
#endif
  const unsigned tiles = (unsigned)((n + tn - 1) / tn);
  const unsigned grid = swz ? 8 * ((tiles + 7) / 8) : tiles;
  if (net.L1 == 3072) {
    hipLaunchKernelGGL((eval_net_kernel<3072, 1>), dim3(grid), dim3(384), 0, s, net, boards, need, n, out, perm, tiles, swz,
                       rows_out, tn, P, nullptr, nullptr);
  } else if (net.L1 == 128) {
    if (cls)
      hipLaunchKernelGGL((eval_net_kernel<128, 16, true>), dim3(grid), dim3(256), 0, s, net, boards, need, n, out, perm,
                         tiles, swz, rows_out, tn, P, need_small, need_big);
    else
      hipLaunchKernelGGL((eval_net_kernel<128, 16>), dim3(grid), dim3(256), 0, s, net, boards, need, n, out, perm, tiles,
                         swz, rows_out, tn, P, nullptr, nullptr);
  } else if (net.L1 == 1024) {
    hipLaunchKernelGGL((eval_net_kernel<1024, 1>), dim3(grid), dim3(128), 0, s, net, boards, need, n, out, perm, tiles, swz,
                       rows_out, tn, P, nullptr, nullptr);
  } else {
    return hipErrorInvalidValue;
  }
  return hipGetLastError();
}

__global__ void classify_kernel(const gn_board *__restrict__ boards, size_t n, gn_eval_params P,
                                uint8_t *__restrict__ need_small, uint8_t *__restrict__ need_big) {
  const size_t i = (size_t)blockIdx.x * blockDim.x + threadIdx.x;
  if (i >= n) return;
  Board B;
  uint8_t s = 0, b = 0;
  if (unpack_fields(boards[i], B)) {
    const Material m = material(B, P);
    const int us = B.stm;
    const int simple = P.piece_value[0] * (m.pawns[us] - m.pawns[us ^ 1]) + (m.npm[us] - m.npm[us ^ 1]);
    s = abs(simple) > P.small_net_threshold;
    b = !s;
  }
  need_small[i] = s;
  need_big[i] = b;
}

__global__ void reeval_kernel(const int2 *__restrict__ out_small, const uint8_t *__restrict__ need_small, size_t n,
                              gn_eval_params P, uint8_t *__restrict__ need_big) {
  const size_t i = (size_t)blockIdx.x * blockDim.x + threadIdx.x;
  if (i >= n || !need_small[i]) return;
  const int2 o = out_small[i];
  const int32_t nnue = wadd(wmul(P.psqt_weight, o.x), wmul(P.positional_weight, o.y)) / 128;
  if (abs(nnue) < P.reeval_threshold) need_big[i] = 1;
}

template <bool CHILD>
__global__ void finalize_kernel(const gn_board *__restrict__ boards, size_t n, int mode,
                                const int2 *__restrict__ out_small, const int2 *__restrict__ out_big,
                                const uint8_t *__restrict__ need_small, const uint8_t *__restrict__ need_big,
                                gn_eval_params P, const Tables *__restrict__ tables, gn_eval *__restrict__ out,
                                const uint32_t *__restrict__ owner, const uint16_t *__restrict__ moves,
                                const Board *__restrict__ unpacked, int score, const uint64_t *__restrict__ counts,
                                NetDevice bnet, const int32_t *__restrict__ part, const int2 *__restrict__ pinfo,
                                uint64_t npos, uint64_t qoff) {
  __shared__ Tables T;
  __shared__ int4v w1s[8 * 32 * 2];
  if (part) stage_fc1(w1s, bnet);
  load_tables(T, tables);
  const size_t stride = (size_t)gridDim.x * blockDim.x;
  for (size_t i = (size_t)blockIdx.x * blockDim.x + threadIdx.x; i < n; i += stride) {
#ifdef GN_AB_FIN_LATE_SUMS
    auto big_out = [&](size_t j) -> int2 {
      if (part) {
        const int2 info = pinfo[qoff + j];
        if (info.y >= 0) return slice_finish_one<GN_PART_SLICES>(bnet, w1s, part, npos, qoff + j, info);
      }
      return out_big[j];
    };
    const uint32_t ow = CHILD ? owner[i] : 0u;
    const uint16_t mv = CHILD ? moves[i] : (uint16_t)0;
#else
    const uint32_t ow = CHILD ? owner[i] : 0u;
    const uint16_t mv = CHILD ? moves[i] : (uint16_t)0;
    int2 info = make_int2(0, -1);
    int4v sums[4];
    if (part) {
      info = pinfo[qoff + i];
      if (mode == GN_MODE_BIG || (mode == GN_MODE_FULL && need_big[i])) slice_sums<GN_PART_SLICES>(part, npos, qoff + i, sums);
    }
    auto big_out = [&](size_t j) -> int2 {
      return part && info.y >= 0 ? slice_finish_from(bnet, w1s, sums, info) : out_big[j];
    };
#endif
    Board B;
    gn_eval e = {0, 0, 0, 0, 0, 0, 0};
    if constexpr (CHILD) {
      B = do_move(unpacked[ow], mv, nullptr);
    } else if (!unpack(boards[i], B, T)) {
      e.flags = GN_FLAG_BAD_FEN | GN_FLAG_NO_SCORE;
      out[i] = e;
      continue;
    }
    const Material m = material(B, P);
    bool small;
    int2 o;
    uint32_t flags = 0;
    if (mode == GN_MODE_SMALL) {
      small = true, o = out_small[i];
    } else if (mode == GN_MODE_BIG) {
      small = false, o = big_out(i);
    } else if (need_small[i] && !need_big[i]) {
      small = true, o = out_small[i];
    } else {
      small = false, o = big_out(i);
      if (need_small[i]) flags |= GN_FLAG_REEVAL;
    }
    int32_t nnue = wadd(wmul(P.psqt_weight, o.x), wmul(P.positional_weight, o.y)) / 128;
    const int32_t complexity = abs(wadd(o.x, -o.y));
    nnue = wadd(nnue, -(wmul(nnue, complexity) / (small ? P.complexity_div_small : P.complexity_div_big)));
    const int32_t mat = (small ? P.material_pawn_small : P.material_pawn_big) * (m.pawns[0] + m.pawns[1]) +
                        m.npm[0] + m.npm[1];
    int32_t v = wmul(nnue, P.material_base + mat) / P.material_base;
    v = wadd(v, -(wmul(v, (int32_t)B.rule50) / P.rule50_div));
    v = clampi(v, -P.value_clamp, P.value_clamp);
    if (small) flags |= GN_FLAG_SMALLNET;
    const bool check = in_check(B, T);
    if (check) flags |= GN_FLAG_IN_CHECK;
    e.psqt = o.x, e.positional = o.y, e.final_v = v;
    e.final_cp = wdl_to_cp(v, wdl_material(B, P), P);
    if (!score) {
      flags |= GN_FLAG_NO_SCORE;
    } else if (counts ? counts[i] == 0 : !any_legal(B, T)) {
      flags |= GN_FLAG_NO_MOVES | (check ? GN_FLAG_MATE : 0u);
    } else {
      e.score = e.final_cp;
    }
    e.flags = (uint16_t)flags;
    out[i] = e;
  }
}

__global__ void score_select_kernel(const gn_eval *__restrict__ out, size_t n, uint64_t *__restrict__ sel) {
  const size_t i = (size_t)blockIdx.x * blockDim.x + threadIdx.x;
  if (i > n) return;
  uint64_t v = 0;
  if (i < n) {
    const uint32_t f = out[i].flags;
    v = (f & GN_FLAG_IN_CHECK) && !(f & (GN_FLAG_NO_MOVES | GN_FLAG_NO_SCORE | GN_FLAG_BAD_FEN));
  }
  sel[i] = v;
}

__global__ void score_gather_kernel(const gn_board *__restrict__ boards, const uint64_t *__restrict__ sel,
                                    const uint64_t *__restrict__ pos, size_t n, const Tables *__restrict__ tables,
                                    uint32_t *__restrict__ idx, gn_board *__restrict__ sb) {
  const size_t i = (size_t)blockIdx.x * blockDim.x + threadIdx.x;
  if (i >= n || !sel[i]) return;
  const uint64_t k = pos[i];
  idx[k] = (uint32_t)i;
  gn_board b = boards[i];
  if (tables) {
    Board B;
    const bool ok = unpack(b, B, *tables);
    b = gn_board{};
    if (ok) pack(B, b);
  }
  sb[k] = b;
}

__global__ void score_counts_kernel(const uint32_t *__restrict__ idx, size_t m, const uint64_t *__restrict__ off,
                                    uint64_t *__restrict__ counts) {
// ... 142 lines not shown
        const uint32_t mv = moves[c + lane];
        const gn_eval r = rec[c + lane];
        const Board C = do_move(B, (uint16_t)mv, nullptr);
        const uint32_t check = (r.flags & GN_FLAG_IN_CHECK) ? 1u : 0u;
        const uint32_t none = any_legal(C, T) ? 0u : 1u;
        const int32_t v = negate_ply(none ? (check ? -VALUE_MATE : 0) : r.final_v);
        key = (uint64_t)(uint32_t)(v + 32768) << 18 | (uint64_t)(0xFFFFu - mv) << 2 | none << 1 | check;
      }
      uint64_t next = 0;
      for (int k = 0; k < K; ++k) {
        const uint64_t mine = key > top ? key : top;
        const uint64_t m = group_max(mine);
        if (!m) break;
        if (key == m) key = 0;
        if (top == m) top = 0;
        if (lane == k) next = m;
      }
      top = next;
    }
    if (lane < K) {
      gn_line l = {0, 0, 0, (uint16_t)GN_FLAG_NO_SCORE};
      if (top) {
        uint32_t fl = ((top & 1) ? GN_FLAG_IN_CHECK : 0u) | ((top & 2) ? GN_FLAG_NO_MOVES : 0u);
        l.value = (int32_t)(top >> 18) - 32768;
        l.move = (uint16_t)(0xFFFFu - (uint32_t)((top >> 2) & 0xFFFFu));
        l.score = rule_score(l.value, wdl_material(B, P), P, fl);
        l.flags = (uint16_t)fl;
      }
      lines[p * (size_t)K + lane] = l;
    }
  }
}

template <class Parent, class Off>
static hipError_t rank_children_t(const Parent *parents, size_t n, const Off *offsets, const uint16_t *moves,
                                  const gn_eval *rec, const gn_eval_params &P, const Tables *tables, int K,
                                  gn_line *lines, hipStream_t s) {
  if (!n) return hipSuccess;
  constexpr size_t per_wg = RANK_WG / GN_RANK_WIDTH, max_blocks = 8192;
  const size_t blocks = std::min<size_t>((n + per_wg - 1) / per_wg, max_blocks);
  hipLaunchKernelGGL((rank_children_kernel<Parent, Off>), dim3(blocks), dim3(RANK_WG), 0, s, parents, n, offsets, moves,
                     rec, P, tables, K, lines);
  return hipGetLastError();
}
hipError_t launch_rank_children(const Board *unpacked, size_t n, const uint64_t *offsets, const uint16_t *moves,
                                const gn_eval *rec, const gn_eval_params &P, const Tables *tables, int K,
                                gn_line *lines, hipStream_t s) {
  return rank_children_t(unpacked, n, offsets, moves, rec, P, tables, K, lines, s);
}
hipError_t launch_rank_children(const gn_board *parents, size_t n, const uint32_t *offsets, const uint16_t *moves,
                                const gn_eval *rec, const gn_eval_params &P, const Tables *tables, int K,
                                gn_line *lines, hipStream_t s) {
  return rank_children_t(parents, n, offsets, moves, rec, P, tables, K, lines, s);
}

hipError_t launch_classify(const gn_board *boards, size_t n, const gn_eval_params &P, uint8_t *need_small,
                           uint8_t *need_big, hipStream_t s) {
  if (!n) return hipSuccess;
  hipLaunchKernelGGL(classify_kernel, dim3(blocks_for(n, 256)), dim3(256), 0, s, boards, n, P, need_small, need_big);
  return hipGetLastError();
}

hipError_t launch_reeval(const int2 *out_small, const uint8_t *need_small, size_t n, const gn_eval_params &P,
                         uint8_t *need_big, hipStream_t s) {
  if (!n) return hipSuccess;
  hipLaunchKernelGGL(reeval_kernel, dim3(blocks_for(n, 256)), dim3(256), 0, s, out_small, need_small, n, P, need_big);
  return hipGetLastError();
}

hipError_t launch_finalize(const gn_board *boards, size_t n, int mode, const int2 *out_small, const int2 *out_big,
                           const uint8_t *need_small, const uint8_t *need_big, const gn_eval_params &P,
                           const Tables *tables, gn_eval *out, hipStream_t s, int score, const uint64_t *counts,
                           const uint32_t *owner, const uint16_t *moves, const Board *unpacked,
                           const SlicedOut *sliced) {
  if (!n) return hipSuccess;
  NetDevice bnet = {};
  if (sliced) bnet = *sliced->net;
  constexpr size_t max_blocks = 8192;
  const size_t blocks = std::min<size_t>(blocks_for(n, 256), max_blocks);
  auto launch = [&](auto kernel) {
    hipLaunchKernelGGL(kernel, dim3(blocks), dim3(256), 0, s, boards, n, mode, out_small, out_big, need_small,
                       need_big, P, tables, out, owner, moves, unpacked, score, counts, bnet,
                       sliced ? sliced->part : nullptr, sliced ? sliced->pinfo : nullptr, sliced ? sliced->npos : 0,
                       sliced ? sliced->qoff : 0);
  };
  if (unpacked) launch(finalize_kernel<true>);
  else launch(finalize_kernel<false>);
  return hipGetLastError();
}

hipError_t launch_score_select(const gn_eval *out, size_t n, uint64_t *sel, hipStream_t s) {
  hipLaunchKernelGGL(score_select_kernel, dim3(blocks_for(n + 1, 256)), dim3(256), 0, s, out, n, sel);
  return hipGetLastError();
}

hipError_t launch_score_gather(const gn_board *boards, const uint64_t *sel, const uint64_t *pos, size_t n,
                               const Tables *tables, uint32_t *idx, gn_board *sb, hipStream_t s) {
  if (!n) return hipSuccess;
  hipLaunchKernelGGL(score_gather_kernel, dim3(blocks_for(n, 256)), dim3(256), 0, s, boards, sel, pos, n, tables, idx, sb);
  return hipGetLastError();
}

hipError_t launch_score_replies(const uint32_t *idx, size_t m, const uint64_t *off, uint64_t *counts,
                                uint64_t *coff, void *&temp, size_t &temp_bytes, uint64_t *total_host, hipStream_t s) {
  hipError_t e;
  hipLaunchKernelGGL(score_counts_kernel, dim3(blocks_for(m + 1, 256)), dim3(256), 0, s, idx, m, off, counts);
  if ((e = hipGetLastError()) != hipSuccess) return e;
  if ((e = exclusive_scan_u64(counts, coff, m + 1, temp, temp_bytes, s)) != hipSuccess) return e;
  if ((e = hipMemcpyAsync(total_host, coff + m, sizeof(uint64_t), hipMemcpyDeviceToHost, s)) != hipSuccess) return e;
  return hipStreamSynchronize(s);
}

hipError_t launch_score_replies_fill(const uint32_t *idx, size_t m, const uint64_t *off, const uint64_t *coff,
                                     const gn_eval *rec, const uint16_t *moves, const Board *unpacked,
                                     const Tables *tables, gn_eval *ce, gn_board *cb, uint16_t *cm, hipStream_t s) {
  if (!m) return hipSuccess;
  hipLaunchKernelGGL(score_replies_kernel, dim3(blocks_for(m, 256)), dim3(256), 0, s, idx, m, off, coff, rec, moves,
                     unpacked, tables, ce, cb, cm);
  return hipGetLastError();
}

#ifndef GN_RL_THREADS
#define GN_RL_THREADS 512
#endif
__device__ __forceinline__ bool level_board(const gn_board &b, Board &B, const Tables &T, int first) {
  return first ? unpack(b, B, T) : unpack_fields(b, B);
}
__global__ void __launch_bounds__(GN_RL_THREADS) reply_level_kernel(const gn_board *__restrict__ boards, uint32_t n,
                                                           const Tables *__restrict__ tables, uint64_t *__restrict__ off,
                                                           uint32_t cap, gn_board *__restrict__ rb,
                                                           uint16_t *__restrict__ rm, uint32_t *__restrict__ flag,
                                                           int first) {
  constexpr uint32_t NT = GN_RL_THREADS, MAXM = 16384 / NT;
  __shared__ Tables T;
  __shared__ uint32_t part[NT];
  __shared__ uint16_t smv[NT][MAXM];
  __shared__ uint8_t spos[NT][MAXM];
  load_tables(T, tables);
  const uint32_t t = threadIdx.x, q = (n + NT - 1) / NT, lo = t * q, hi = lo + q < n ? lo + q : n;
  uint32_t c = 0;
#pragma unroll 1
  for (uint32_t i = lo; i < hi; ++i) {
    uint32_t cnt = 0;
    Board B;
    if (level_board(boards[i], B, T, first) && in_check(B, T))
      gen_legal(B, T, [&](uint16_t m) {
        if (c + cnt < MAXM) smv[t][c + cnt] = m, spos[t][c + cnt] = (uint8_t)(i - lo);
        ++cnt;
      });
    off[i] = cnt;
    c += cnt;
  }
  part[t] = c;
  __syncthreads();
  for (uint32_t d = 1; d < NT; d <<= 1) {
    const uint32_t v = t >= d ? part[t - d] : 0u;
    __syncthreads();
    part[t] += v;
    __syncthreads();
  }
  const uint32_t total = part[NT - 1];
  uint32_t base = part[t] - c;
  const bool spill = c > MAXM;
#pragma unroll 1
  for (uint32_t i = lo; i < hi; ++i) {
    const uint32_t cnt = (uint32_t)off[i];
    off[i] = base < cap ? base : cap;
// ... 500 lines not shown
```

fishnet_amd/csrc/nnue.h:

```cpp
#pragma once
#include <stdint.h>

#include "chess.h"

namespace gn {

constexpr int FT_INPUTS = 22528;
constexpr int FT_BIAS_ROW = FT_INPUTS;
constexpr int FT_ROWS = FT_INPUTS + 1;
#ifndef GN_ROW_ALIGN
#define GN_ROW_ALIGN 128
#endif
constexpr uint32_t ft_row_stride(uint32_t l1) { return (2 * l1 + 32 + GN_ROW_ALIGN - 1) / GN_ROW_ALIGN * GN_ROW_ALIGN; }
constexpr int CARRY_SLOTS = 2048;
constexpr int CARRY_ROW0 = FT_ROWS;
constexpr int KC_ROW0 = CARRY_ROW0 + 4 * CARRY_SLOTS;
static_assert(KC_ROW0 + 128 * CARRY_SLOTS <= (1 << 19), "carry and king-cache rows must fit the 19-bit row field");
constexpr int SCR_ROWS = 130;
constexpr int POOL_PER_XCD = 256;
constexpr int SCR_SLOTS = 8 * POOL_PER_XCD;
static_assert(SCR_ROWS * SCR_SLOTS <= 132 * CARRY_SLOTS, "scratch slots fit the rows behind the FT rows");
constexpr int ZERO_ROW = FT_ROWS + 132 * CARRY_SLOTS;
static_assert(ZERO_ROW < (1 << 19), "the zero row fits the 19-bit row field");
constexpr int PSQT_BUCKETS = 8;
constexpr int LAYER_STACKS = 8;
constexpr uint32_t NNUE_VERSION = 0x7AF32F20u;

struct NetDevice {
  int L1;
  uint32_t row_stride;
  int carry_slots;
  int kc_slots;
  const uint8_t *ft;
  const int16_t *bias;
  const int8_t *w0;
  const int32_t *b0;
  const int8_t *w1;
  const int32_t *b1;
  const int8_t *w2;
  const int32_t *b2;
  const int32_t *psqt;
  const int8_t *w0f;
};

GN_HD int feature_index(int persp, int sq, int pc, int ksq) {
  const int kf = ksq & 7;
  const int orient = (kf < 4 ? 7 : 0) ^ (persp ? 56 : 0);
  const int rel_rank = (ksq >> 3) ^ (persp ? 7 : 0);
  const int bucket = 4 * (7 - rel_rank) + (kf < 4 ? kf : 7 - kf);
  const int pt = pc & 7;
  const int plane = pt == KING ? 10 : 2 * (pt - 1) + ((pc >> 3) != persp);
  return (sq ^ orient) + 64 * plane + 704 * bucket;
}

struct ChildDelta {
  uint16_t idx[2][4];
  uint32_t meta;
  uint32_t pad;
};
static_assert(sizeof(ChildDelta) == 24, "ChildDelta is 24 bytes");

GN_HD ChildDelta make_child_delta(const Board &parent, const Board &child, const Dirty &d) {
  ChildDelta cd;
  uint32_t meta = 0;
#pragma unroll
  for (int h = 0; h < 2; ++h) {
    const int ksq = king_square(child, h);
    cd.idx[h][0] = cd.idx[h][1] = cd.idx[h][2] = cd.idx[h][3] = 0;
    if (d.king_moved && h == parent.stm) {
      meta |= 1u << (8 + h);
      const bool castle = d.n_add == 2;
      cd.idx[h][0] = (uint16_t)d.rem_sq[0];
      cd.idx[h][1] = (uint16_t)d.add_sq[0];
      cd.idx[h][2] = (uint16_t)(castle ? d.rem_sq[1] : 64);
      cd.idx[h][3] = (uint16_t)(castle ? d.add_sq[1] : 64);
    } else {
      cd.idx[h][0] = (uint16_t)feature_index(h, d.rem_sq[0], d.rem_pc[0], ksq);
      if (d.n_rem > 1) cd.idx[h][1] = (uint16_t)feature_index(h, d.rem_sq[1], d.rem_pc[1], ksq);
      cd.idx[h][2] = (uint16_t)feature_index(h, d.add_sq[0], d.add_pc[0], ksq);
      if (d.n_add > 1) cd.idx[h][3] = (uint16_t)feature_index(h, d.add_sq[1], d.add_pc[1], ksq);
      meta |= (uint32_t)(d.n_rem | (d.n_add << 2)) << (4 * h);
    }
  }
  meta |= (uint32_t)child.stm << 10;
  meta |= (uint32_t)((popcnt(child.byType[0]) - 1) / 4) << 11;
  meta |= (uint32_t)popcnt(child.byType[0]) << 14;
// ... 81 lines not shown
```

fishnet_amd/csrc/stream.hip:

```cpp
#include <stdio.h>
#include <stdlib.h>
#include <string.h>

#include <type_traits>

#include "device_util.h"
#include "kernels.h"

#ifndef GN_PLAN_WPE
#define GN_PLAN_WPE 4
#endif
#ifndef GN_SLICE_WPE
#define GN_SLICE_WPE 4
#endif
#define GN_PART_N GN_PART_SLICES
#ifndef GN_WCACHE
#define GN_WCACHE 1
#endif
#ifndef GN_EXPAND_WPE
#define GN_EXPAND_WPE (GN_RING == 4 ? 5 : 4)
#endif
#define GN_STR2(x) #x
#define GN_STR(x) GN_STR2(x)

// ... 528 lines not shown
          ps::wave_sync();
        }
        if (kuse) {
          uint32_t &sf = g ? safe1 : safe0;
          sf = base + (uint32_t)ne - 1 + GN_SCR_GAP;
        }
        if (g) len1 += (uint32_t)ne;
        else len0 += (uint32_t)ne;
      }
      while (jc < ntp - 1) close_tile(jc), ++jc, open_tile(jc);
      pp_d += PP_T() - pp_t, pp_t = PP_T();
      {
        const uint32_t rel = exc - (uint32_t)__shfl((int)exc, tile_lane0(tix));
        const uint32_t at0 = (uint32_t)__shfl((int)ts0, tix) + (rel & 0xFFFF);
        const uint32_t at1 = (uint32_t)__shfl((int)ts1, tix) + (rel >> 16);
        const uint32_t t0w = hs(t, cst != 0, xu, hu), t1w = hs(t, cst != 1, xu, hu);
        if (in && live) {
          auto delta = [&](int g, uint32_t at, uint32_t lo2, uint32_t hi2, int s, int n, bool hit, uint32_t tw,
                           uint32_t L) {
            const uint32_t i0 = lo2 & 0xFFFF, i1 = lo2 >> 16, i2 = hi2 & 0xFFFF, i3 = hi2 >> 16;
            auto cl = [](uint32_t r) { return (r < (uint32_t)FT_INPUTS ? r : (uint32_t)FT_BIAS_ROW) * RS; };
            const uint32_t r1 = cl(s >= 2 ? i1 : i2), r2 = cl(s >= 2 ? i2 : i3), r3 = cl(i3);
            const uint32_t f1 = s >= 2 ? M_SUB : M_ADD;
            if (!hit) {
              put(g, at, cl(i0), M_SUB | HP | tw | (n == 1 ? L : 0u));
              if (n > 1) put(g, at + 1, r1, f1 | tw | (n == 2 ? L : 0u));
              if (n > 2) put(g, at + 2, r2, M_ADD | tw | (n == 3 ? L : 0u));
              if (n > 3) put(g, at + 3, r3, M_ADD | tw | L);
            } else {
              put(g, at, r1, f1 | HB | tw | (n == 2 ? L : 0u));
              if (n > 2) put(g, at + 1, r2, M_ADD | tw | (n == 3 ? L : 0u));
              if (n > 3) put(g, at + 2, r3, M_ADD | tw | L);
            }
          };
          if ((kinds & 3) == 1) delta(0, at0, w0, w1, s0, n0, hit0, t0w, H_LAST | (nx ? H_PAR_E : 0u));
          if ((kinds >> 2) == 1) delta(1, at1, w2, w3, s1, n1, hit1, t1w, H_LAST | (nx ? H_PAR_E : 0u));
        }
      }
      uint32_t lbm = 0;
#pragma unroll
      for (int b = 0; b < 8; ++b)
        if (__ballot(tix == ntp - 1 && ((mybit >> b) & 1))) lbm |= 1u << b;
      if (ntp > 1) p_first = p, t_first = u_fill + (uint32_t)tile_lane0(ntp - 1);
      tile_k = tk0 + (uint32_t)(ntp - 1);
      t_fill = ntp == 1 ? tf0 + n_in : n_in - tile_lane0(ntp - 1);
      tile_bm = ntp == 1 ? tile_bm | lbm : lbm;
      u_fill += (uint32_t)n_in;
      pp_c += PP_T() - pp_t;
      if (t_fill == 16) flush();
    }
  }
  if (t_fill) flush();
#ifdef GN_FAULT_PLAN_BLOCK
  if (blk == (uint32_t)(GN_FAULT_PLAN_BLOCK) && tile_k > 0) {
    int armed = lane == 0 ? atomicExch(&gn_fault_armed, 0) : 0;
    if (__builtin_amdgcn_readfirstlane(armed)) {
      if (lane == 0) *reinterpret_cast<uint2 *>(tf(tile_k - 1, 0)) = make_uint2(rtot + 4096u, rtot + 4096u);
      bad |= 1u;
    }
  }
#endif
  if (lane == 0) btiles[blk] = tile_k;
  const uint32_t werr = __ballot(bad & 1u) ? 1u : 0u, werr4 = __ballot(bad & 4u) ? 4u : 0u;
  if (lane == 0) {
    if ((uint64_t)len0 + len1 > (uint64_t)(rtot - ENT_SPARE) || werr) atomicOr(err, 1u);
    if (werr4) atomicOr(err, 4u);
    if (rows_out) atomicAdd(rows_out, (unsigned long long)rows);
    if (pads_out && pads) atomicAdd(pads_out, (unsigned long long)pads);
    PP_ADD(0, pp_a), PP_ADD(1, pp_b), PP_ADD(2, pp_c), PP_ADD(3, pp_d);
    SP_ADD(6, pads), SP_ADD(7, fpads);
  }
  (void)pads, (void)fpads;
}

template <int L1, int SL = 1>
__global__ void __launch_bounds__(L1 / SL / 8) __attribute__((amdgpu_waves_per_eu(SL > 1 ? GN_SLICE_WPE : GN_EXPAND_WPE)))
    stream_eval_kernel(NetDevice net, const uint64_t *__restrict__ offsets, uint32_t np, uint32_t K, uint32_t b0,
                       uint32_t b1, int swz,
                       const uint64_t *__restrict__ eoff, const uint64_t *__restrict__ ent,
                       const TileDesc *__restrict__ tiles, const uint32_t *__restrict__ btiles,
                       const uint32_t *__restrict__ order, int2 *__restrict__ out_parent, int2 *__restrict__ out_child,
                       uint32_t *__restrict__ pool, int use_scr, uint32_t *__restrict__ err,
                       uint32_t *__restrict__ claim, int slice, int32_t *__restrict__ part, uint64_t npos,
                       int2 *__restrict__ pinfo) {
  using namespace ps;
  constexpr int LC = L1 / SL;
  constexpr int G = LC / 16;
  constexpr int NT = 2 * G, NW = NT / 64, TILE = 16, XS = tile_xs(L1, SL), KS = LC / 64,
                KPW = KS / NW;
  constexpr int KSF = L1 / 64;
  constexpr uint32_t RS = ft_row_stride(L1);
  static_assert(G % 64 == 0 && KS % NW == 0 && KPW % 2 == 0 && L1 % SL == 0, "geometry");
  const uint32_t cofs = SL > 1 ? (uint32_t)slice * (uint32_t)LC : 0u;
  __shared__ __attribute__((aligned(16))) uint8_t xt[TILE * XS];
  constexpr int AS = 20;
  __shared__ __attribute__((aligned(16))) int32_t acc0[2][16 * AS];
  __shared__ __attribute__((aligned(16))) uint8_t in1[2][TILE][32];
  __shared__ int32_t fwd[2][TILE];
  __shared__ uint32_t sslot, sblk;
  const int tid = threadIdx.x;
  const int wave = __builtin_amdgcn_readfirstlane(tid >> 6);
  const int hu = __builtin_amdgcn_readfirstlane((tid / G) & 1);
  for (int i = tid; i < 2 * 16 * AS; i += NT) (&acc0[0][0])[i] = 0;
  const uint32_t nblk = b1 - b0;
  const uint32_t vgrid = swz == 1 ? 8 * ((nblk + 7) / 8) : nblk;
  uint32_t v = blockIdx.x;
  if (swz == 0) {
    if (tid == 0) sblk = atomicAdd(claim, 1u);
    __syncthreads();
    v = sblk;
  } else if (swz == 2) {
    if (tid == 0) {
      uint32_t x;
      asm volatile("s_getreg_b32 %0, hwreg(HW_REG_XCC_ID)" : "=s"(x));
      x &= 7;
      const uint32_t per = (nblk + 7) / 8;
      uint32_t got = ~0u;
      for (uint32_t t = 0; t < 8 && got == ~0u; ++t) {
        const uint32_t y = (x + t) & 7, lo = y * per, hi = lo + per < nblk ? lo + per : nblk;
        if (lo >= hi || __hip_atomic_load(claim + y, __ATOMIC_RELAXED, __HIP_MEMORY_SCOPE_AGENT) >= hi - lo) continue;
        const uint32_t i = atomicAdd(claim + y, 1u);
        if (i < hi - lo) got = lo + i;
      }
      sblk = got;
    }
    __syncthreads();
    v = sblk;
  }
  if (v >= vgrid) return;
  uint32_t blk = v;
  if (swz == 1) {
    const uint32_t b8 = (nblk + 7) / 8;
    blk = (v & 7) * b8 + (v >> 3);
    if (blk >= nblk) return;
  }
  blk = order ? order[b0 + blk] : blk + b0;
  const uint32_t pbeg = blk * K, pend = pbeg + K < np ? pbeg + K : np;
  const uint64_t us_b = pbeg + offsets[pbeg];
  const uint32_t ntiles = btiles[blk];
  const TileDesc *T = tiles + us_b / 16 + (uint64_t)(K + 2) * blk;
  const uint64_t rbeg = eoff[pbeg] + (uint64_t)ENT_SPARE * blk, rend = eoff[pend] + (uint64_t)ENT_SPARE * (blk + 1);
  const uint32_t elim = (uint32_t)(rend - rbeg) - ENT_SPARE;
#ifdef GN_XCD_PROF
  const unsigned long long xp_t0 = __builtin_amdgcn_s_memrealtime();
#endif
  uint32_t scr = 0, my_slot = 0;
  if (use_scr) {
    if (tid == 0) {
      uint32_t x;
      asm volatile("s_getreg_b32 %0, hwreg(HW_REG_XCC_ID)" : "=s"(x));
      x &= 7;
      uint32_t *wd = pool + 8 * x;
      int got = -1;
      for (int it = 0; it < 4096 && got < 0; ++it) {
        const int wi = (int)((it + (v >> 3)) & 7);
        uint32_t cur = __hip_atomic_load(wd + wi, __ATOMIC_RELAXED, __HIP_MEMORY_SCOPE_AGENT);
        while (cur != 0xFFFFFFFFu) {
          const int bit = __builtin_ctz(~cur);
          const uint32_t old = __hip_atomic_fetch_or(wd + wi, 1u << bit, __ATOMIC_RELAXED, __HIP_MEMORY_SCOPE_AGENT);
          if (!(old & (1u << bit))) {
            got = (int)(x * POOL_PER_XCD + 32 * wi + bit);
            break;
          }
          cur = old | (1u << bit);
        }
        if (got < 0 && wi == 7) __builtin_amdgcn_s_sleep(4);
      }
// ... 343 lines not shown
    }
    uint32_t mm = SL > 1 && ((bm >> cb) & 1) ? (bm ^ (1u << cb)) | 256u : bm;
#pragma unroll 1
    while (mm) {
      int b;
      if (mm & 256u) b = cb, mm ^= 256u;
      else b = __builtin_ctz(mm), mm &= mm - 1;
      const int buf = (int)(bq & 1);
      int tl = tid;
      asm volatile("" : "+v"(tl));
      const int ln = tl & 63, row = ln & 15, kg = ln >> 4;
      if constexpr (SL > 1 && GN_WCACHE) {
        if (b != cb) {
          cb = b;
          wc_load(b);
          GN_WC_WAIT(0);
        }
        const uint8_t *xa = xt + row * XS + kg * 16 + 64 * KPW * wave;
        int4v acc = {0, 0, 0, 0};
        constexpr int FB = 2;
        int stop = 0;
        asm volatile("" : "+s"(stop));
#pragma unroll
        for (int k0 = 0; k0 < KPW && !stop; k0 += FB) {
          int4v av[FB];
#pragma unroll
          for (int j = 0; j < FB; ++j) av[j] = *reinterpret_cast<const int4v *>(xa + 64 * (k0 + j));
#pragma unroll
          for (int j = 0; j < FB; ++j) acc = __builtin_amdgcn_mfma_i32_16x16x64_i8(av[j], wc[k0 + j], acc, 0, 0, 0);
        }
#pragma unroll
        for (int i = 0; i < 4; ++i) atomicAdd(&acc0[buf][(4 * kg + i) * AS + row], acc[i]);
      } else {
        const uint8_t *xa = xt + row * XS + kg * 16 + 64 * KPW * wave;
        constexpr int WH = NW / 2;
        const int wsl = SL > 1 ? (wave / WH) * WH * SL + slice * WH + wave % WH : wave;
#ifdef GN_AB_W0_FIXED
        const int8_t *wb = net.w0f + (size_t)ln * 16;
        constexpr int WSTEP = 0;
#else
        const int8_t *wb = net.w0f + (((size_t)b * KSF + KPW * wsl) * 64 + ln) * 16;
        constexpr int WSTEP = 1024;
#endif
        int4v acc = {0, 0, 0, 0};
        constexpr int FB = 2;
        int stop = 0;
        asm volatile("" : "+s"(stop));
#pragma unroll
        for (int k0 = 0; k0 < KPW && !stop; k0 += FB) {
          int4v wv[FB], av[FB];
#pragma unroll
          for (int j = 0; j < FB; ++j) wv[j] = *reinterpret_cast<const int4v *>(wb + WSTEP * (k0 + j));
#pragma unroll
          for (int j = 0; j < FB; ++j) av[j] = *reinterpret_cast<const int4v *>(xa + 64 * (k0 + j));
#pragma unroll
          for (int j = 0; j < FB; ++j) acc = __builtin_amdgcn_mfma_i32_16x16x64_i8(av[j], wv[j], acc, 0, 0, 0);
        }
#pragma unroll
        for (int i = 0; i < 4; ++i) atomicAdd(&acc0[buf][(4 * kg + i) * AS + row], acc[i]);
      }
#ifndef GN_AB_NO_BARRIER
      __syncthreads();
#endif
      auto present = [&](int pos) -> bool {
        const uint32_t m = (mw[pos >> 2] >> (8 * (pos & 3))) & 0xFF;
        return (m & 1) && (int)((m >> 1) & 7) == b;
      };
      auto out_index = [&](int pos, int adjv) -> uint64_t {
        const uint32_t P = p_first + (uint32_t)__builtin_popcount(pm & ((2u << pos) - 1)) - (pm & 1);
        return ((pm >> pos) & 1) ? (uint64_t)P : (uint64_t)np + (u0 + pos - P - 1 + adjv);
      };
      if constexpr (SL > 1) {
        if (wave == (int)(bq % NW)) {
          const int wp = ln >> 2, wj = ln & 3;
          const int adjv = adj_of(D, wp);
          int4v *src = reinterpret_cast<int4v *>(&acc0[buf][wp * AS + 4 * wj]);
          if (present(wp)) {
            const uint64_t q = out_index(wp, adjv);
            int4v v = *src;
            if (GN_PART_N == 1 && slice > 0) {
#pragma unroll
              for (int k = 0; k < 4; ++k) v[k] = wadd(v[k], pv[k]);
            }
            *reinterpret_cast<int4v *>(part + ((uint64_t)(GN_PART_N == 1 ? 0 : slice) * npos + q) * 16 + 4 * wj) = v;
          }
          *src = int4v{0, 0, 0, 0};
        }
      } else if (wave == (int)(bq % NW)) {
        const int32_t bias0 = net.b0[b * 16 + row];
        const int32_t b1l = net.b1[b * 32 + row], b1h = net.b1[b * 32 + 16 + row];
        const int32_t w2l = net.w2[b * 32 + row], w2h = net.w2[b * 32 + 16 + row];
        const int32_t b2v = net.b2[b];
        int2 pq[4] = {};
        int adj[4] = {};
        if (row == 0) {
#pragma unroll
          for (int i = 0; i < 4; ++i) pq[i] = *reinterpret_cast<const int2 *>(D->psq[4 * kg + i]), adj[i] = D->adj[4 * kg + i];
        }
#pragma unroll
        for (int i = 0; i < 4; ++i) {
          const int pos = 4 * kg + i;
          const int32_t vv = wadd(acc0[buf][pos * AS + row], bias0);
          if (row < 15) {
            const long long s2 = ((long long)vv * vv) >> 19;
            in1[buf][pos][row] = (uint8_t)(s2 < 127 ? s2 : 127);
            in1[buf][pos][15 + row] = (uint8_t)clampi(vv >> 6, 0, 127);
          } else {
            fwd[buf][pos] = wmul(vv, 600 * 16) / (127 * 64);
            in1[buf][pos][30] = 0;
            in1[buf][pos][31] = 0;
          }
        }
        ps::wave_sync();
#pragma unroll
        for (int i = 0; i < 4; ++i) acc0[buf][(4 * kg + i) * AS + row] = 0;
        const int4v zero = {0, 0, 0, 0};
        const int4v wl = *reinterpret_cast<const int4v *>(net.w1 + ((size_t)b * 32 + row) * 32 + (kg & 1) * 16);
        const int4v wh = *reinterpret_cast<const int4v *>(net.w1 + ((size_t)b * 32 + 16 + row) * 32 + (kg & 1) * 16);
        int4v a1 = zero;
        if (kg < 2) a1 = *reinterpret_cast<const int4v *>(&in1[buf][row][kg * 16]);
        const int4v cl = __builtin_amdgcn_mfma_i32_16x16x64_i8(a1, wl, zero, 0, 0, 0);
        const int4v ch = __builtin_amdgcn_mfma_i32_16x16x64_i8(a1, wh, zero, 0, 0, 0);
        int32_t l2[4];
#pragma unroll
        for (int i = 0; i < 4; ++i) {
          const int32_t l = clampi(wadd(cl[i], b1l) >> 6, 0, 127), hh = clampi(wadd(ch[i], b1h) >> 6, 0, 127);
          l2[i] = w2l * l + w2h * hh;
        }
#pragma unroll
        for (int off = 8; off; off >>= 1)
#pragma unroll
          for (int i = 0; i < 4; ++i) l2[i] = wadd(l2[i], __shfl_xor(l2[i], off, 16));
        if (row == 0) {
#pragma unroll
          for (int i = 0; i < 4; ++i) {
            const int pos = 4 * kg + i;
            const uint32_t m = (mw[pos >> 2] >> (8 * (pos & 3))) & 0xFF;
            if ((m & 1) && (int)((m >> 1) & 7) == b) {
              const int32_t positional = wadd(wadd(b2v, l2[i]), fwd[buf][pos]);
              const int32_t psqt = (int32_t)((uint32_t)pq[i].x - (uint32_t)pq[i].y) / 2;
              const int2 val = make_int2(psqt / 16, positional / 16);
              const uint32_t P = p_first + (uint32_t)__builtin_popcount(pm & ((2u << pos) - 1)) - (pm & 1);
              if ((pm >> pos) & 1) out_parent[P] = val;
              else out_child[u0 + pos - P - 1 + adj[i]] = val;
            }
          }
        }
      }
      ++bq;
    }
    sp_l += SP_T() - t2;
  }
#ifdef GN_STREAM_PROF
  if ((tid & 63) == 0) {
    SP_ADD(0, sp_s), SP_ADD(1, sp_w), SP_ADD(2, sp_l);
    if (wave == 0) SP_ADD(3, ntiles), SP_ADD(4, sp_m), SP_ADD(5, sp_n);
  }
#else
  (void)sp_s, (void)sp_w, (void)sp_l, (void)sp_m, (void)sp_n, (void)sp_e0, (void)sp_e1;
#endif
  };
  if (hu) run_group(std::integral_constant<int, 1>{});
  else run_group(std::integral_constant<int, 0>{});
  if (use_scr) {
    asm volatile("s_waitcnt vmcnt(0)" ::: "memory");
    __syncthreads();
    if (tid == 0)
      __hip_atomic_fetch_and(pool + 8 * (my_slot / POOL_PER_XCD) + (my_slot % POOL_PER_XCD) / 32,
                             ~(1u << (my_slot % 32)), __ATOMIC_RELAXED, __HIP_MEMORY_SCOPE_AGENT);
  }
#ifdef GN_XCD_PROF
  if (tid == 0) {
    uint32_t x;
    asm volatile("s_getreg_b32 %0, hwreg(HW_REG_XCC_ID)" : "=s"(x));
    x &= 7;
    const unsigned long long t1 = __builtin_amdgcn_s_memrealtime();
    atomicMax(&gn_xp[x], t1);
    atomicMin(&gn_xp[8 + x], xp_t0);
    atomicAdd(&gn_xp[16 + x], ntiles ? (unsigned long long)T[ntiles - 1].e_end[0] + T[ntiles - 1].e_end[1] : 0ull);
    atomicAdd(&gn_xp[24 + x], 1ull);
  }
#endif
}

template <int SL>
__global__ void __launch_bounds__(256) slice_finish_kernel(NetDevice net, const int32_t *__restrict__ part,
                                                           const int2 *__restrict__ pinfo, uint64_t npos, uint32_t np,
                                                           int2 *__restrict__ out_parent, int2 *__restrict__ out_child) {
  __shared__ int4v w1s[8 * 32 * 2];
  stage_fc1(w1s, net);
  __syncthreads();
  const uint64_t q = (uint64_t)blockIdx.x * blockDim.x + threadIdx.x;
  if (q >= npos) return;
  const int2 info = pinfo[q];
  if (info.y < 0) return;
  const int2 val = slice_finish_one<GN_PART_N>(net, w1s, part, npos, q, info);
  if (q < np) out_parent[q] = val;
  else out_child[q - np] = val;
}

hipError_t launch_plan_stream(const NetDevice &net, const PlanStreamArgs &a, int phases, hipStream_t s) {
  const size_t n = a.n;
  if (!n) return hipSuccess;
  const bool do_plan = phases & PLAN_PHASE, do_stream = phases & STREAM_PHASE;
  if (n >= 0x80000000ull) return hipErrorInvalidValue;
  const uint32_t K = a.chain_k > 1 && a.next_slot ? (uint32_t)a.chain_k : 1u;
  const uint8_t *next_slot = K > 1 ? a.next_slot : nullptr;
  const int kc = K > 1 ? a.kc : 0;
  const int scr = K > 1 && a.kc;
  const uint32_t nb = (uint32_t)((n + K - 1) / K), B0 = 0, B1 = nb;
  const unsigned pg = (nb + PLAN_WAVES - 1) / PLAN_WAVES, g = a.swz == 1 ? 8 * ((nb + 7) / 8) : nb + nb / 16 + 8;
  auto stream_done = [&] {
    if (a.fin) (void)hipEventRecord(a.fin, s);
    if (a.streamed) (void)hipEventRecord(a.streamed, s);
  };
  if (net.L1 == 3072) {
    const bool sliced = a.slices == 3 && a.part && a.pinfo;
    if (do_plan) {
      if (sliced) {
        hipError_t e = hipMemsetAsync(a.pinfo, 0xFF, a.npos * sizeof(int2), s);
        if (e != hipSuccess) return e;
      }
      hipLaunchKernelGGL((plan_kernel<3072>), dim3(pg), dim3(GN_FRONT_WG), 0, s, net, a.parents, a.offsets, a.deltas,
                         a.need_parent, a.need_child, next_slot, (uint32_t)n, K, B0, B1, kc, a.eoff, a.ent, a.tiles,
                         a.btiles, a.rows_out, a.pads_out, a.err, sliced ? a.pinfo : nullptr,
                         sliced ? ps::field_xu(3072, 3) : ps::field_xu(3072, 1), sliced ? ps::field_hu(3072, 3) : ps::field_hu(3072, 1));
      if (a.mid) (void)hipEventRecord(a.mid, s);
    }
    if (!do_stream) {
    } else if (sliced) {
      for (int sl = 0; sl < 3; ++sl)
        hipLaunchKernelGGL((stream_eval_kernel<3072, 3>), dim3(g), dim3(128), 0, s, net, a.offsets, (uint32_t)n, K, B0,
                           B1, a.swz, a.eoff, a.ent, a.tiles, a.btiles, a.order, a.out_parent, a.out_child, a.pool, scr,
                           a.err, a.pool + 64 + 8 * sl, sl, a.part, (uint64_t)a.npos, a.pinfo);
      stream_done();
      if (a.finish)
        hipLaunchKernelGGL((slice_finish_kernel<3>), dim3((unsigned)((a.npos + 255) / 256)), dim3(256), 0, s, net,
                           a.part, a.pinfo, (uint64_t)a.npos, (uint32_t)n, a.out_parent, a.out_child);
    } else {
      hipLaunchKernelGGL((stream_eval_kernel<3072>), dim3(g), dim3(384), 0, s, net, a.offsets, (uint32_t)n, K, B0, B1,
                         a.swz, a.eoff, a.ent, a.tiles, a.btiles, a.order, a.out_parent, a.out_child, a.pool, scr, a.err,
                         a.pool + 64, 0, nullptr, (uint64_t)0, nullptr);
      stream_done();
    }
  } else if (net.L1 == 1024) {
    if (do_plan) {
      hipLaunchKernelGGL((plan_kernel<1024>), dim3(pg), dim3(GN_FRONT_WG), 0, s, net, a.parents, a.offsets, a.deltas,
                         a.need_parent, a.need_child, next_slot, (uint32_t)n, K, B0, B1, kc, a.eoff, a.ent, a.tiles,
                         a.btiles, a.rows_out, a.pads_out, a.err, nullptr, ps::field_xu(1024, 1), ps::field_hu(1024, 1));
      if (a.mid) (void)hipEventRecord(a.mid, s);
    }
    if (do_stream) {
      hipLaunchKernelGGL((stream_eval_kernel<1024>), dim3(g), dim3(128), 0, s, net, a.offsets, (uint32_t)n, K, B0, B1,
                         a.swz, a.eoff, a.ent, a.tiles, a.btiles, a.order, a.out_parent, a.out_child, a.pool, scr, a.err,
                         a.pool + 64, 0, nullptr, (uint64_t)0, nullptr);
      stream_done();
    }
  } else {
    return hipErrorInvalidValue;
  }
#ifdef GN_PLAN_PROF
  {
    unsigned long long c[4];
    (void)hipStreamSynchronize(s);
    (void)hipMemcpyFromSymbol(c, HIP_SYMBOL(gn_pp), sizeof(c));
    fprintf(stderr, "plan prof: wave-cycles setup %llu slots %llu delta puts %llu king jobs %llu\n", c[0], c[1],
            c[2], c[3]);
    memset(c, 0, sizeof(c));
    (void)hipMemcpyToSymbol(HIP_SYMBOL(gn_pp), c, sizeof(c));
  }
#endif
#ifdef GN_XCD_PROF
  {
    unsigned long long c[32];
    (void)hipStreamSynchronize(s);
    (void)hipMemcpyFromSymbol(c, HIP_SYMBOL(gn_xp), sizeof(c));
    unsigned long long t0 = ~0ull;
    for (int x = 0; x < 8; ++x) t0 = c[8 + x] < t0 ? c[8 + x] : t0;
    fprintf(stderr, "xcd prof:");
    for (int x = 0; x < 8; ++x)
      fprintf(stderr, " [%d] end %.2f ms start %.2f ms entries %llu wgs %llu;", x, (c[x] - t0) * 1e-5,
              (c[8 + x] - t0) * 1e-5, c[16 + x], c[24 + x]);
    fprintf(stderr, "\n");
    for (int x = 0; x < 8; ++x) c[x] = 0, c[8 + x] = ~0ull, c[16 + x] = 0, c[24 + x] = 0;
    (void)hipMemcpyToSymbol(HIP_SYMBOL(gn_xp), c, sizeof(c));
  }
#endif
#ifdef GN_STREAM_PROF
  {
    unsigned long long c[8];
    (void)hipStreamSynchronize(s);
    (void)hipMemcpyFromSymbol(c, HIP_SYMBOL(gn_sp), sizeof(c));
    fprintf(stderr, "stream prof: wave-cycles stream %llu barrier %llu ls %llu; tiles %llu; "
                    "entries max-list %llu sum %llu (balance %.3f), no-op entries %llu scratch-order + %llu tile-end\n",
            c[0], c[1], c[2], c[3], c[4], c[5], c[5] ? 2.0 * c[4] / c[5] : 0.0, c[6], c[7]);
    memset(c, 0, sizeof(c));
    (void)hipMemcpyToSymbol(HIP_SYMBOL(gn_sp), c, sizeof(c));
  }
#endif
  return hipGetLastError();
}

}
```

fishnet_amd/gpu_nnue.py:

```python
from __future__ import annotations

import ctypes as C
import os

import numpy as np

HERE = os.path.dirname(os.path.abspath(__file__))
LIB_PATH = os.environ.get("GPU_NNUE_LIB", os.path.join(HERE, "lib", "libgpu_nnue.so"))

MODE_FULL, MODE_BIG, MODE_SMALL = 0, 1, 2
FLAG_IN_CHECK, FLAG_SMALLNET, FLAG_BAD_FEN, FLAG_REEVAL, FLAG_SKIPPED = 1, 2, 4, 8, 16
FLAG_MATE, FLAG_NO_SCORE, FLAG_SEARCHED, FLAG_NO_MOVES = 32, 64, 128, 256
ERRORS = {-1: "INVALID", -2: "IO", -3: "FORMAT", -4: "HIP", -5: "NOMEM", -6: "CAPACITY",
          -7: "NODEVICE", -8: "NONET", -9: "ILLEGAL_MOVE"}
E_INVALID, E_IO, E_FORMAT, E_HIP, E_NOMEM, E_CAPACITY, E_NODEVICE, E_NONET, E_ILLEGAL_MOVE = -1, -2, -3, -4, -5, -6, -7, -8, -9

EVAL_DTYPE = np.dtype([("psqt", "<i4"), ("positional", "<i4"), ("final_v", "<i4"), ("final_cp", "<i4"),
                       ("score", "<i4"), ("flags", "<u2"), ("best_move", "<u2")])
BOARD_DTYPE = np.dtype([("occ", "<u8"), ("pc", "u1", (16,)), ("stm_ep", "u1"), ("reserved", "u1"),
                        ("castle", "<u2"), ("rule50", "<u2"), ("fullmove", "<u2")])
CHILD_DTYPE = np.dtype([("psqt", "<i4"), ("positional", "<i4"), ("cp_flags", "<i4")])
CHILD_VIEW_DTYPE = np.dtype([("psqt", "<i4"), ("positional", "<i4"), ("final_cp", "<i4"), ("flags", "<u2")])
LINE_DTYPE = np.dtype([("value", "<i4"), ("score", "<i4"), ("move", "<u2"), ("flags", "<u2")])
MAX_LINES = 8
EVAL_SIZE, BOARD_SIZE, CHILD_SIZE = EVAL_DTYPE.itemsize, BOARD_DTYPE.itemsize, CHILD_DTYPE.itemsize
assert EVAL_SIZE == 24 and BOARD_SIZE == 32 and CHILD_SIZE == 12 and LINE_DTYPE.itemsize == 12
ABI_VERSION = 4

EXPORTS = ["gn_load_net", "gn_load_net_memory", "gn_free", "gn_last_error", "gn_abi_version",
           "gn_get_eval_params", "gn_set_eval_params", "gn_net_info", "gn_evaluate_batch",
           "gn_evaluate_batch_mode", "gn_expand_and_evaluate", "gn_perft", "gn_pack_fens",
           "gn_board_to_fen", "gn_random_positions", "gn_evaluate_device", "gn_expand_device",
           "gn_device_alloc", "gn_device_free", "gn_memcpy_h2d", "gn_memcpy_d2h", "gn_synchronize",
           "gn_time_evaluate_device", "gn_random_positions_device", "gn_set_option", "gn_get_option",
           "gn_time_expand_device", "gn_random_games_device", "gn_replay_game", "gn_evaluate_games",
           "gn_net_sha256", "gn_partition", "gn_checksum_device",
           "gn_boards_to_fens", "gn_load_net_archive", "gn_archive_read", "gn_expand2_device",
           "gn_random_games_uci", "gn_rank_children_device", "gn_evaluate_games_lines"]
OPT_INCREMENTAL_CHILDREN, OPT_XCD_SWIZZLE, OPT_KING_SORT, OPT_CHAIN, OPT_KING_CACHE = 1, 2, 3, 4, 5
OPT_CHUNK_PARENTS, OPT_COALESCE, OPT_STREAM_SLICES, OPT_FAST_BATCH, OPT_EXPAND_PIPELINE = 6, 7, 8, 9, 10
STAT_PLAN_NS, STAT_STREAM_NS, STAT_SCRATCH_PADS, STAT_FINISH_NS = 101, 102, 103, 104
STAT_BATCH_LAUNCHES, STAT_BATCH_CALLS, STAT_FAST_BATCHES, STAT_FAST_FALLBACKS = 117, 118, 119, 120
STAT_RANK_NS = 121
HOST_STAGES = {"parse": 110, "upload": 111, "replay": 112, "compute": 113, "download": 114, "tail": 115, "total": 116}
EXPAND_STAGES = ["count_scan", "total_readback", "write_children", "classify", "small_net", "big_net", "finalize",
                 "score"]


def decode_children(raw) -> np.ndarray:
    raw = np.asarray(raw, dtype=CHILD_DTYPE)
    out = np.empty(raw.shape, dtype=CHILD_VIEW_DTYPE)
    cf = raw["cp_flags"].astype(np.int64)
    out["psqt"], out["positional"] = raw["psqt"], raw["positional"]
    out["final_cp"] = ((cf & 0xFFFFFF) ^ 0x800000) - 0x800000
    out["flags"] = (cf >> 24) & 0xFF
    return out


def children_from_evals(ev) -> np.ndarray:
    ev = np.asarray(ev, dtype=EVAL_DTYPE)
    out = np.empty(ev.shape, dtype=CHILD_VIEW_DTYPE)
    out["psqt"], out["positional"], out["final_cp"] = ev["psqt"], ev["positional"], ev["final_cp"]
    out["flags"] = ev["flags"] & 0xFF
    return out


class GnError(RuntimeError):
    def __init__(self, code, msg):
        super().__init__(f"gpu_nnue error {code} ({ERRORS.get(code, '?')}): {msg}")
        self.code = code


class EvalParams(C.Structure):
    _fields_ = [(n, C.c_int32) for n in (
        "small_net_threshold", "psqt_weight", "positional_weight", "reeval_threshold",
        "complexity_div_small", "complexity_div_big", "material_pawn_small", "material_pawn_big",
        "material_base", "rule50_div", "value_clamp")] + [
        ("piece_value", C.c_int32 * 5), ("wdl_a", C.c_double * 4), ("wdl_material_min", C.c_int32),
        ("wdl_material_max", C.c_int32), ("wdl_material_anchor", C.c_int32), ("wdl_piece_weight", C.c_int32 * 5)]


class GnGame(C.Structure):
    _fields_ = [("root_fen", C.c_char_p), ("uci_moves", C.c_char_p),
                ("skip_positions", C.POINTER(C.c_uint32)), ("n_skip", C.c_size_t)]


def _games_array(games):
    keep, arr = [], (GnGame * max(len(games), 1))()
    for i, g in enumerate(games):
        root, moves, skip = (tuple(g) + ((),) * 3)[:3]
        mv = moves if isinstance(moves, str) else " ".join(moves or ())
        sk = (C.c_uint32 * max(len(skip), 1))(*skip)
        keep += [root.encode(), mv.encode(), sk]
        arr[i].root_fen, arr[i].uci_moves = keep[-3], keep[-2]
        arr[i].skip_positions = C.cast(sk, C.POINTER(C.c_uint32))
        arr[i].n_skip = len(skip)
    return arr, keep


_lib = None


def lib():
    global _lib
    if _lib is not None:
        return _lib
    if not os.path.exists(LIB_PATH):
        raise ImportError(f"libgpu_nnue.so not built at {LIB_PATH}: run `python -m fishnet_amd.build`")
    L = C.CDLL(LIB_PATH)
    vp, sz, i32 = C.c_void_p, C.c_size_t, C.c_int
    sig = {
        "gn_load_net": [C.c_char_p, C.c_char_p, vp, i32, C.POINTER(vp)],
        "gn_load_net_memory": [vp, sz, vp, sz, vp, i32, C.POINTER(vp)],
        "gn_free": [vp],
        "gn_last_error": [],
        "gn_abi_version": [],
        "gn_get_eval_params": [vp, C.POINTER(EvalParams)],
        "gn_set_eval_params": [vp, C.POINTER(EvalParams)],
        "gn_net_info": [vp, C.POINTER(i32), C.POINTER(C.c_uint32), C.POINTER(i32), C.POINTER(C.c_uint32)],
        "gn_evaluate_batch": [vp, vp, sz, vp],
        "gn_evaluate_batch_mode": [vp, vp, sz, i32, vp],
        "gn_expand_and_evaluate": [vp, vp, sz, i32, vp, vp, vp, vp, sz],
        "gn_perft": [vp, C.c_char_p, i32, C.POINTER(C.c_uint64)],
        "gn_pack_fens": [vp, sz, vp, vp],
        "gn_board_to_fen": [vp, C.c_char_p, sz],
        "gn_random_positions": [C.c_uint64, sz, sz, i32, vp],
# ... 411 lines not shown
```

include/gpu_nnue.h:

```cpp
#ifndef GPU_NNUE_H
#define GPU_NNUE_H
#include <stddef.h>
#include <stdint.h>

#ifdef __cplusplus
extern "C" {
#endif

#define GN_ABI_VERSION 4

#if defined(__GNUC__)
#define GN_API __attribute__((visibility("default")))
#else
#define GN_API
#endif

#define GN_OK 0
#define GN_E_INVALID (-1)
#define GN_E_IO (-2)
#define GN_E_FORMAT (-3)
#define GN_E_HIP (-4)
#define GN_E_NOMEM (-5)
#define GN_E_CAPACITY (-6)
#define GN_E_NODEVICE (-7)
#define GN_E_NONET (-8)
#define GN_E_ILLEGAL_MOVE (-9)

#define GN_MODE_FULL 0
#define GN_MODE_BIG 1
#define GN_MODE_SMALL 2

#define GN_OPT_CHUNK_PARENTS 6
#define GN_OPT_COALESCE 7
#define GN_OPT_FAST_BATCH 9
#define GN_OPT_EXPAND_PIPELINE 10
#define GN_OPT_INCREMENTAL_CHILDREN 1
#define GN_OPT_XCD_SWIZZLE 2
#define GN_OPT_KING_SORT 3
#define GN_OPT_KING_CACHE 5
#define GN_OPT_CHAIN 4
#define GN_OPT_STREAM_SLICES 8

#define GN_STAT_PLAN_NS 101
#define GN_STAT_STREAM_NS 102
#define GN_STAT_FINISH_NS 104
#define GN_STAT_SCRATCH_PADS 103
#define GN_STAT_HOST_PARSE_NS 110
#define GN_STAT_HOST_UPLOAD_NS 111
#define GN_STAT_HOST_REPLAY_NS 112
#define GN_STAT_HOST_COMPUTE_NS 113
#define GN_STAT_HOST_DOWNLOAD_NS 114
#define GN_STAT_HOST_TAIL_NS 115
#define GN_STAT_HOST_TOTAL_NS 116
#define GN_STAT_RANK_NS 121
#define GN_STAT_BATCH_LAUNCHES 117
#define GN_STAT_BATCH_CALLS 118
#define GN_STAT_FAST_BATCHES 119
#define GN_STAT_FAST_FALLBACKS 120

#define GN_FLAG_IN_CHECK 1u
#define GN_FLAG_SMALLNET 2u
#define GN_FLAG_BAD_FEN 4u
#define GN_FLAG_REEVAL 8u
#define GN_FLAG_SKIPPED 16u
#define GN_FLAG_MATE 32u
#define GN_FLAG_NO_SCORE 64u
#define GN_FLAG_SEARCHED 128u
#define GN_FLAG_NO_MOVES 256u

typedef struct gn_eval {
  int32_t psqt;
  int32_t positional;
  int32_t final_v;
  int32_t final_cp;
  int32_t score;
  uint16_t flags;
  uint16_t best_move;
} gn_eval;

typedef struct gn_child {
  int32_t psqt;
  int32_t positional;
  int32_t cp_flags;
} gn_child;
#define GN_CHILD_FINAL_CP(c) ((int32_t)((uint32_t)(c).cp_flags << 8) >> 8)
#define GN_CHILD_FLAGS(c) ((uint32_t)(c).cp_flags >> 24)

#define GN_MAX_LINES 8
typedef struct gn_line {
  int32_t value;
  int32_t score;
  uint16_t move;
  uint16_t flags;
} gn_line;

typedef struct gn_board {
  uint64_t occ;
  uint8_t pc[16];
  uint8_t stm_ep;
  uint8_t reserved;
  uint16_t castle;
  uint16_t rule50;
  uint16_t fullmove;
} gn_board;

typedef struct gn_eval_params {
  int32_t small_net_threshold;
  int32_t psqt_weight;
  int32_t positional_weight;
  int32_t reeval_threshold;
  int32_t complexity_div_small;
  int32_t complexity_div_big;
  int32_t material_pawn_small;
  int32_t material_pawn_big;
  int32_t material_base;
  int32_t rule50_div;
  int32_t value_clamp;
  int32_t piece_value[5];
  double wdl_a[4];
  int32_t wdl_material_min;
  int32_t wdl_material_max;
  int32_t wdl_material_anchor;
  int32_t wdl_piece_weight[5];
} gn_eval_params;

typedef struct gn_ctx gn_ctx;

GN_API int gn_load_net(const char *big_path, const char *small_path, const int *devices, int n_devices,
                gn_ctx **out);
GN_API int gn_load_net_memory(const uint8_t *big, size_t big_len, const uint8_t *small, size_t small_len,
                       const int *devices, int n_devices, gn_ctx **out);
GN_API int gn_load_net_archive(const char *archive_path, const char *big_member, const char *small_member,
                               const int *devices, int n_devices, gn_ctx **out);
GN_API int gn_archive_read(const char *archive_path, const char *member, uint8_t *buf, size_t cap, size_t *size);
GN_API void gn_free(gn_ctx *ctx);
GN_API const char *gn_last_error(void);
GN_API int gn_abi_version(void);
// ... 78 lines not shown
```

rust/gpu-nnue-sys/src/lib.rs:

```rust
#![allow(non_camel_case_types)]
use std::os::raw::{c_char, c_int, c_void};

pub const GN_ABI_VERSION: c_int = 4;

pub const GN_OK: c_int = 0;
pub const GN_E_INVALID: c_int = -1;
pub const GN_E_IO: c_int = -2;
pub const GN_E_FORMAT: c_int = -3;
pub const GN_E_HIP: c_int = -4;
pub const GN_E_NOMEM: c_int = -5;
pub const GN_E_CAPACITY: c_int = -6;
pub const GN_E_NODEVICE: c_int = -7;
pub const GN_E_NONET: c_int = -8;
pub const GN_E_ILLEGAL_MOVE: c_int = -9;

pub const GN_MODE_FULL: c_int = 0;
pub const GN_MODE_BIG: c_int = 1;
pub const GN_MODE_SMALL: c_int = 2;

pub const GN_OPT_INCREMENTAL_CHILDREN: c_int = 1;
pub const GN_OPT_XCD_SWIZZLE: c_int = 2;
pub const GN_OPT_KING_SORT: c_int = 3;
pub const GN_OPT_CHAIN: c_int = 4;
pub const GN_OPT_KING_CACHE: c_int = 5;
pub const GN_OPT_CHUNK_PARENTS: c_int = 6;
pub const GN_OPT_COALESCE: c_int = 7;
pub const GN_OPT_STREAM_SLICES: c_int = 8;
pub const GN_OPT_FAST_BATCH: c_int = 9;
pub const GN_OPT_EXPAND_PIPELINE: c_int = 10;
pub const GN_STAT_PLAN_NS: c_int = 101;
pub const GN_STAT_STREAM_NS: c_int = 102;
pub const GN_STAT_SCRATCH_PADS: c_int = 103;
pub const GN_STAT_FINISH_NS: c_int = 104;
pub const GN_STAT_HOST_PARSE_NS: c_int = 110;
pub const GN_STAT_HOST_UPLOAD_NS: c_int = 111;
pub const GN_STAT_HOST_REPLAY_NS: c_int = 112;
pub const GN_STAT_HOST_COMPUTE_NS: c_int = 113;
pub const GN_STAT_HOST_DOWNLOAD_NS: c_int = 114;
pub const GN_STAT_HOST_TAIL_NS: c_int = 115;
pub const GN_STAT_HOST_TOTAL_NS: c_int = 116;
pub const GN_STAT_BATCH_LAUNCHES: c_int = 117;
pub const GN_STAT_BATCH_CALLS: c_int = 118;
pub const GN_STAT_FAST_BATCHES: c_int = 119;
pub const GN_STAT_FAST_FALLBACKS: c_int = 120;
pub const GN_STAT_RANK_NS: c_int = 121;

pub const GN_FLAG_IN_CHECK: u16 = 1;
pub const GN_FLAG_SMALLNET: u16 = 2;
pub const GN_FLAG_BAD_FEN: u16 = 4;
pub const GN_FLAG_REEVAL: u16 = 8;
pub const GN_FLAG_SKIPPED: u16 = 16;
pub const GN_FLAG_MATE: u16 = 32;
pub const GN_FLAG_NO_SCORE: u16 = 64;
pub const GN_FLAG_SEARCHED: u16 = 128;
pub const GN_FLAG_NO_MOVES: u16 = 256;

#[repr(C)]
#[derive(Clone, Copy, Default, Debug, PartialEq, Eq)]
pub struct gn_eval {
    pub psqt: i32,
    pub positional: i32,
    pub final_v: i32,
    pub final_cp: i32,
    pub score: i32,
    pub flags: u16,
    pub best_move: u16,
}

#[repr(C)]
#[derive(Clone, Copy, Default, Debug, PartialEq, Eq)]
pub struct gn_child {
    pub psqt: i32,
    pub positional: i32,
    pub cp_flags: i32,
}

impl gn_child {
    pub fn final_cp(&self) -> i32 {
        ((self.cp_flags as u32) << 8) as i32 >> 8
    }
    pub fn flags(&self) -> u16 {
        ((self.cp_flags as u32) >> 24) as u16
    }
}

pub const MAX_LINES: usize = 8;

#[repr(C)]
#[derive(Clone, Copy, Default, Debug, PartialEq, Eq)]
pub struct gn_line {
    pub value: i32,
    pub score: i32,
    pub r#move: u16,
    pub flags: u16,
}

#[repr(C)]
#[derive(Clone, Copy, Default, Debug, PartialEq, Eq)]
pub struct gn_board {
    pub occ: u64,
    pub pc: [u8; 16],
    pub stm_ep: u8,
    pub reserved: u8,
    pub castle: u16,
    pub rule50: u16,
    pub fullmove: u16,
}

#[repr(C)]
#[derive(Clone, Copy, Default, Debug, PartialEq)]
pub struct gn_eval_params {
    pub small_net_threshold: i32,
    pub psqt_weight: i32,
    pub positional_weight: i32,
    pub reeval_threshold: i32,
    pub complexity_div_small: i32,
    pub complexity_div_big: i32,
    pub material_pawn_small: i32,
    pub material_pawn_big: i32,
    pub material_base: i32,
    pub rule50_div: i32,
    pub value_clamp: i32,
    pub piece_value: [i32; 5],
    pub wdl_a: [f64; 4],
    pub wdl_material_min: i32,
    pub wdl_material_max: i32,
    pub wdl_material_anchor: i32,
    pub wdl_piece_weight: [i32; 5],
// ... 112 lines not shown
```

Before: 852.1 million.

## Pack sliced partial fc0 sums into 24-bit records when weight bounds allow

Adds a packed 48-byte partial-sum record format for the 3-slice big-net path, replacing the 64-byte int32 layout. Each of the 16 partial sums fits in 24 bits, which the host verifies at load time by bounding the fc0 weight magnitudes against the 7-bit clipped FT inputs. The stream kernel writes records with an inline-asm dwordx3 store, and the finish and finalize kernels unpack them with perm and sign-extend. This cuts intermediate HBM write and read traffic and scratch size by a quarter, at the cost of extra pack/unpack ALU work and a fallback path when the bound check fails.

```diff
diff --git a/fishnet_amd/build.py b/fishnet_amd/build.py
--- a/fishnet_amd/build.py
+++ b/fishnet_amd/build.py
@@ -14,7 +14,8 @@
 ODD_LIB = os.path.join(LIBDIR, "libgpu_nnue_d5.so")
 ODD_DEFINES = ("-DGN_SMALL_DEPTH=5",)
 SOURCES = ["gpu_nnue.hip", "kernels.hip", "stream.hip"]
-HEADERS = ["chess.h", "host_board.h", "nnue.h", "kernels.h", "sha256.h", "device_util.h", "archive.h"]
+HEADERS = ["chess.h", "host_board.h", "nnue.h", "kernels.h", "sha256.h", "device_util.h", "archive.h",
+           "part_format.h"]
 ARCH = "gfx950"
 
 
diff --git a/fishnet_amd/csrc/device_util.h b/fishnet_amd/csrc/device_util.h
--- a/fishnet_amd/csrc/device_util.h
+++ b/fishnet_amd/csrc/device_util.h
@@ -103,14 +103,14 @@
 typedef unsigned short ushort2v __attribute__((ext_vector_type(2)));
 __device__ __forceinline__ uint2 transform8(ushort8 lo, ushort8 hi) {
   uint32_t o[4];
-  const short2v z = {0, 0}, m = {254, 254};
+  const short2v z = {0, 0}, m = {FT_CLIP, FT_CLIP};
 #pragma unroll
   for (int i = 0; i < 4; ++i) {
     short2v a = {(short)lo[2 * i], (short)lo[2 * i + 1]}, b = {(short)hi[2 * i], (short)hi[2 * i + 1]};
     a = __builtin_elementwise_min(__builtin_elementwise_max(a, z), m);
     b = __builtin_elementwise_min(__builtin_elementwise_max(b, z), m);
     ushort2v pr = __builtin_bit_cast(ushort2v, a) * __builtin_bit_cast(ushort2v, b);
-    pr = pr >> (ushort2v){9, 9};
+    pr = pr >> (ushort2v){FT_PAIR_SHIFT, FT_PAIR_SHIFT};
     o[i] = __builtin_bit_cast(uint32_t, pr);
   }
   return make_uint2(__builtin_amdgcn_perm(o[1], o[0], 0x06040200u), __builtin_amdgcn_perm(o[3], o[2], 0x06040200u));
@@ -250,8 +250,39 @@
 __device__ __forceinline__ void stage_fc1(int4v *w1s, const NetDevice &net) {
   for (int i = threadIdx.x; i < 8 * 32 * 2; i += blockDim.x) w1s[i] = reinterpret_cast<const int4v *>(net.w1)[i];
 }
+typedef int int3v __attribute__((ext_vector_type(3)));
+__device__ __forceinline__ int3v pack_sums24(int4v v, uint32_t sel = 0x04020100u) {
+  return int3v{(int)__builtin_amdgcn_perm((uint32_t)v[3], (uint32_t)v[0], sel),
+               (int)__builtin_amdgcn_perm((uint32_t)v[3], (uint32_t)v[1], sel + 0x01000000u),
+               (int)__builtin_amdgcn_perm((uint32_t)v[3], (uint32_t)v[2], sel + 0x02000000u)};
+}
+__device__ __forceinline__ int4v unpack_sums24(int32_t d0, int32_t d1, int32_t d2) {
+  const uint32_t lo = __builtin_amdgcn_perm((uint32_t)d1, (uint32_t)d0, 0x0c0c0703u);
+  auto sx24 = [](int32_t d) { return (int32_t)((uint32_t)d << 8) >> 8; };
+  return int4v{sx24(d0), sx24(d1), sx24(d2), (int32_t)(((uint32_t)(d2 >> 24) << 16) | lo)};
+}
 template <int NPART>
-__device__ __forceinline__ void slice_sums(const int32_t *__restrict__ part, uint64_t npos, uint64_t q, int4v (&sums)[4]) {
+__device__ __forceinline__ void slice_sums(const int32_t *__restrict__ part, uint64_t npos, uint64_t q, int4v (&sums)[4],
+                                           bool packed) {
+  if (packed) {
+    int4v w[NPART][3];
+#pragma unroll
+    for (int t = 0; t < NPART; ++t)
+#pragma unroll
+      for (int r = 0; r < 3; ++r) w[t][r] = *reinterpret_cast<const int4v *>(part + ((uint64_t)t * npos + q) * 12 + 4 * r);
+#pragma unroll
+    for (int t = 0; t < NPART; ++t) {
+      const int32_t d[12] = {w[t][0][0], w[t][0][1], w[t][0][2], w[t][0][3], w[t][1][0], w[t][1][1],
+                             w[t][1][2], w[t][1][3], w[t][2][0], w[t][2][1], w[t][2][2], w[t][2][3]};
+#pragma unroll
+      for (int g = 0; g < 4; ++g) {
+        const int4v c = unpack_sums24(d[3 * g], d[3 * g + 1], d[3 * g + 2]);
+#pragma unroll
+        for (int k = 0; k < 4; ++k) sums[g][k] = t ? wadd(sums[g][k], c[k]) : c[k];
+      }
+    }
+    return;
+  }
 #pragma unroll
   for (int r = 0; r < 4; ++r) {
     sums[r] = *reinterpret_cast<const int4v *>(part + q * 16 + 4 * r);
@@ -295,9 +326,9 @@
 }
 template <int NPART>
 __device__ __forceinline__ int2 slice_finish_one(const NetDevice &net, const int4v *w1s, const int32_t *__restrict__ part,
-                                                 uint64_t npos, uint64_t q, int2 info) {
+                                                 uint64_t npos, uint64_t q, int2 info, bool packed) {
   int4v sums[4];
-  slice_sums<NPART>(part, npos, q, sums);
+  slice_sums<NPART>(part, npos, q, sums, packed);
   return slice_finish_from(net, w1s, sums, info);
 }
 
diff --git a/fishnet_amd/csrc/gpu_nnue.hip b/fishnet_amd/csrc/gpu_nnue.hip
--- a/fishnet_amd/csrc/gpu_nnue.hip
+++ b/fishnet_amd/csrc/gpu_nnue.hip
@@ -265,6 +265,8 @@
   DevBuf<unsigned long long> sum;
   DevBuf<uint8_t> nslot;
   DevBuf<int32_t> part;
+  int part_bytes = 64;
+  size_t part_words(size_t positions) const { return (size_t)GN_PART_SLICES * (part_bytes / 4) * positions; }
   bool part_locked = false;
   DevBuf<uint64_t> ebound;
   DevBuf<uint32_t> pool;
@@ -454,6 +456,8 @@
   n.b2 = reinterpret_cast<const int32_t *>(m + off[7]);
   n.psqt = reinterpret_cast<const int32_t *>(m + off[8]);
   n.w0f = reinterpret_cast<const int8_t *>(m + off[9]);
+  if (which == BIG)
+    d.part_bytes = GN_PART_PACK && GN_PART_SLICES == 3 && h.L1 == 3072 ? part_record_bytes(h.w0.data(), LAYER_STACKS * 16, h.L1) : 64;
   d.has[which] = true;
   return GN_OK;
 }
@@ -676,8 +680,8 @@
                         bool score_parents, bool sliced = false) {
   const gn_eval_params &P = ctx->P;
   const ExpSet &x = d.cur;
-  const SlicedOut sc = {&d.net[BIG], d.part.p, x.pinfo.p, (uint64_t)(n + total), (uint64_t)n},
-                  sp = {&d.net[BIG], d.part.p, x.pinfo.p, (uint64_t)(n + total), 0};
+  const SlicedOut sc = {&d.net[BIG], d.part.p, x.pinfo.p, (uint64_t)(n + total), (uint64_t)n, d.part_bytes},
+                  sp = {&d.net[BIG], d.part.p, x.pinfo.p, (uint64_t)(n + total), 0, d.part_bytes};
   const bool fast = x.child_moves != nullptr;
   HIP_TRY(launch_finalize(children, total, mode, x.eb.osm.p, x.eb.obg.p, x.eb.nsm.p, x.eb.nbg.p, P, d.tables, child_out,
                           s, 0, nullptr, fast ? x.owner.p : nullptr, fast ? x.child_moves : nullptr,
@@ -814,7 +818,7 @@
     a.eoff = x.eoff.p, a.ent = x.ent.p, a.tiles = x.tiles.p, a.btiles = x.btiles.p;
     a.pool = d.pool.p, a.err = x.perr.p, a.rows_out = o.rows, a.pads_out = x.pstat.p;
     a.slices = x.slices, a.npos = n + total;
-    if (x.slices > 1) a.part = d.part.p, a.pinfo = x.pinfo.p;
+    if (x.slices > 1) a.part = d.part.p, a.part_bytes = d.part_bytes, a.pinfo = x.pinfo.p;
     return a;
   };
   if (phases & EXP_FRONT) {
@@ -852,7 +856,7 @@
       HIP_TRY(x.btiles.ensure(nblk + 1));
       HIP_TRY(d.pool.ensure(88));
       if (d.net[BIG].L1 == 3072 && ctx->stream_slices == 3) {
-        const size_t need = (size_t)GN_PART_SLICES * 16 * (n + total);
+        const size_t need = d.part_words(n + total);
         bool ok = d.part_locked ? d.part.cap >= need : d.part.ensure(need) == hipSuccess;
         ok = ok && x.pinfo.ensure(n + total) == hipSuccess;
         if (ok) x.slices = 3;
@@ -1367,7 +1371,7 @@
     HIP_TRY(hipStreamWaitEvent(F, d.ev_streamed, 0));
     if (largest) {
       if (d.has[BIG] && d.net[BIG].L1 == 3072 && ctx->stream_slices == 3 &&
-          d.part.ensure((size_t)GN_PART_SLICES * 16 * largest) != hipSuccess)
+          d.part.ensure(d.part_words(largest)) != hipSuccess)
         (void)hipGetLastError();
       d.part_locked = true;
     }
@@ -2678,6 +2682,11 @@
     *value = (int64_t)(m * 1e6);
     return GN_OK;
   }
+  case GN_STAT_PART_BYTES: {
+    const Dev &d = *ctx->devs[0];
+    *value = d.has[BIG] && d.net[BIG].L1 == 3072 && ctx->stream_slices == 3 ? d.part_bytes : 0;
+    return GN_OK;
+  }
   case GN_STAT_SCRATCH_PADS: {
     int64_t sum = 0;
     for (auto &dp : ctx->devs) {
diff --git a/fishnet_amd/csrc/kernels.h b/fishnet_amd/csrc/kernels.h
--- a/fishnet_amd/csrc/kernels.h
+++ b/fishnet_amd/csrc/kernels.h
@@ -25,6 +25,9 @@
 #define GN_PART_SLICES 1
 #else
 #define GN_PART_SLICES 3
+#endif
+#ifndef GN_PART_PACK
+#define GN_PART_PACK 1
 #endif
 
 namespace gn {
@@ -72,6 +75,7 @@
   const uint32_t *order = nullptr;
   int slices = 1;
   int32_t *part = nullptr;
+  int part_bytes = 64;
   size_t npos = 0;
   int2 *pinfo = nullptr;
   bool finish = true;
@@ -89,6 +93,7 @@
   const int32_t *part;
   const int2 *pinfo;
   uint64_t npos, qoff;
+  int part_bytes;
 };
 hipError_t launch_finalize(const gn_board *boards, size_t n, int mode, const int2 *out_small,
                            const int2 *out_big, const uint8_t *need_small, const uint8_t *need_big,
diff --git a/fishnet_amd/csrc/kernels.hip b/fishnet_amd/csrc/kernels.hip
--- a/fishnet_amd/csrc/kernels.hip
+++ b/fishnet_amd/csrc/kernels.hip
@@ -681,7 +681,7 @@
                                 const uint32_t *__restrict__ owner, const uint16_t *__restrict__ moves,
                                 const Board *__restrict__ unpacked, int score, const uint64_t *__restrict__ counts,
                                 NetDevice bnet, const int32_t *__restrict__ part, const int2 *__restrict__ pinfo,
-                                uint64_t npos, uint64_t qoff) {
+                                uint64_t npos, uint64_t qoff, int packed) {
   __shared__ Tables T;
   __shared__ int4v w1s[8 * 32 * 2];
   if (part) stage_fc1(w1s, bnet);
@@ -692,7 +692,7 @@
     auto big_out = [&](size_t j) -> int2 {
       if (part) {
         const int2 info = pinfo[qoff + j];
-        if (info.y >= 0) return slice_finish_one<GN_PART_SLICES>(bnet, w1s, part, npos, qoff + j, info);
+        if (info.y >= 0) return slice_finish_one<GN_PART_SLICES>(bnet, w1s, part, npos, qoff + j, info, packed);
       }
       return out_big[j];
     };
@@ -705,7 +705,7 @@
     int4v sums[4];
     if (part) {
       info = pinfo[qoff + i];
-      if (mode == GN_MODE_BIG || (mode == GN_MODE_FULL && need_big[i])) slice_sums<GN_PART_SLICES>(part, npos, qoff + i, sums);
+      if (mode == GN_MODE_BIG || (mode == GN_MODE_FULL && need_big[i])) slice_sums<GN_PART_SLICES>(part, npos, qoff + i, sums, packed);
     }
     auto big_out = [&](size_t j) -> int2 {
       return part && info.y >= 0 ? slice_finish_from(bnet, w1s, sums, info) : out_big[j];
@@ -1014,7 +1014,7 @@
     hipLaunchKernelGGL(kernel, dim3(blocks), dim3(256), 0, s, boards, n, mode, out_small, out_big, need_small,
                        need_big, P, tables, out, owner, moves, unpacked, score, counts, bnet,
                        sliced ? sliced->part : nullptr, sliced ? sliced->pinfo : nullptr, sliced ? sliced->npos : 0,
-                       sliced ? sliced->qoff : 0);
+                       sliced ? sliced->qoff : 0, sliced && sliced->part_bytes == 48 ? 1 : 0);
   };
   if (unpacked) launch(finalize_kernel<true>);
   else launch(finalize_kernel<false>);
diff --git a/fishnet_amd/csrc/nnue.h b/fishnet_amd/csrc/nnue.h
--- a/fishnet_amd/csrc/nnue.h
+++ b/fishnet_amd/csrc/nnue.h
@@ -2,6 +2,7 @@
 #include <stdint.h>
 
 #include "chess.h"
+#include "part_format.h"
 
 namespace gn {
 
diff --git a/fishnet_amd/csrc/part_format.h b/fishnet_amd/csrc/part_format.h
--- /dev/null
+++ b/fishnet_amd/csrc/part_format.h
@@ -0,0 +1,27 @@
+#pragma once
+#include <stddef.h>
+#include <stdint.h>
+
+namespace gn {
+
+constexpr int FT_CLIP = 254, FT_PAIR_SHIFT = 9;
+constexpr int FC0_IN_MAX = (FT_CLIP * FT_CLIP) >> FT_PAIR_SHIFT;
+static_assert(FC0_IN_MAX == 126, "fc_0 inputs are 7-bit");
+
+inline int part_record_bytes(const int8_t *w0, int rows, int l1) {
+  const int half = l1 / 2, sw = half / 3;
+  for (int r = 0; r < rows; ++r)
+    for (int s = 0; s < 3; ++s) {
+      int64_t p = 0, n = 0;
+      for (int h = 0; h < 2; ++h) {
+        const int8_t *w = w0 + (size_t)r * l1 + (size_t)h * half + (size_t)s * sw;
+        for (int c = 0; c < sw; ++c)
+          if (w[c] > 0) p += w[c];
+          else n -= w[c];
+      }
+      if (FC0_IN_MAX * p > (1 << 23) - 1 || FC0_IN_MAX * n > (1 << 23)) return 64;
+    }
+  return 48;
+}
+
+}
diff --git a/fishnet_amd/csrc/stream.hip b/fishnet_amd/csrc/stream.hip
--- a/fishnet_amd/csrc/stream.hip
+++ b/fishnet_amd/csrc/stream.hip
@@ -634,7 +634,7 @@
                        const uint32_t *__restrict__ order, int2 *__restrict__ out_parent, int2 *__restrict__ out_child,
                        uint32_t *__restrict__ pool, int use_scr, uint32_t *__restrict__ err,
                        uint32_t *__restrict__ claim, int slice, int32_t *__restrict__ part, uint64_t npos,
-                       int2 *__restrict__ pinfo) {
+                       int2 *__restrict__ pinfo, int packed) {
   using namespace ps;
   constexpr int LC = L1 / SL;
   constexpr int G = LC / 16;
@@ -1144,7 +1144,18 @@
 #pragma unroll
               for (int k = 0; k < 4; ++k) v[k] = wadd(v[k], pv[k]);
             }
-            *reinterpret_cast<int4v *>(part + ((uint64_t)(GN_PART_N == 1 ? 0 : slice) * npos + q) * 16 + 4 * wj) = v;
+            const uint64_t rec = (uint64_t)(GN_PART_N == 1 ? 0 : slice) * npos + q;
+            if (GN_PART_N > 1 && packed) {
+              uint32_t sel = 0x04020100u;
+              asm volatile("" : "+s"(sel));
+              asm volatile("global_store_dwordx3 %0, %1, off\n\t"
+                           "s_nop 0"
+                           :
+                           : "v"(part + rec * 12 + 3 * wj), "v"(pack_sums24(v, sel))
+                           : "memory");
+            } else {
+              *reinterpret_cast<int4v *>(part + rec * 16 + 4 * wj) = v;
+            }
           }
           *src = int4v{0, 0, 0, 0};
         }
@@ -1248,7 +1259,8 @@
 template <int SL>
 __global__ void __launch_bounds__(256) slice_finish_kernel(NetDevice net, const int32_t *__restrict__ part,
                                                            const int2 *__restrict__ pinfo, uint64_t npos, uint32_t np,
-                                                           int2 *__restrict__ out_parent, int2 *__restrict__ out_child) {
+                                                           int2 *__restrict__ out_parent, int2 *__restrict__ out_child,
+                                                           int packed) {
   __shared__ int4v w1s[8 * 32 * 2];
   stage_fc1(w1s, net);
   __syncthreads();
@@ -1256,7 +1268,7 @@
   if (q >= npos) return;
   const int2 info = pinfo[q];
   if (info.y < 0) return;
-  const int2 val = slice_finish_one<GN_PART_N>(net, w1s, part, npos, q, info);
+  const int2 val = slice_finish_one<GN_PART_N>(net, w1s, part, npos, q, info, packed);
   if (q < np) out_parent[q] = val;
   else out_child[q - np] = val;
 }
@@ -1278,6 +1290,7 @@
   };
   if (net.L1 == 3072) {
     const bool sliced = a.slices == 3 && a.part && a.pinfo;
+    const int packed = GN_PART_SLICES > 1 && a.part_bytes == 48 ? 1 : 0;
     if (do_plan) {
       if (sliced) {
         hipError_t e = hipMemsetAsync(a.pinfo, 0xFF, a.npos * sizeof(int2), s);
@@ -1294,15 +1307,15 @@
       for (int sl = 0; sl < 3; ++sl)
         hipLaunchKernelGGL((stream_eval_kernel<3072, 3>), dim3(g), dim3(128), 0, s, net, a.offsets, (uint32_t)n, K, B0,
                            B1, a.swz, a.eoff, a.ent, a.tiles, a.btiles, a.order, a.out_parent, a.out_child, a.pool, scr,
-                           a.err, a.pool + 64 + 8 * sl, sl, a.part, (uint64_t)a.npos, a.pinfo);
+                           a.err, a.pool + 64 + 8 * sl, sl, a.part, (uint64_t)a.npos, a.pinfo, packed);
       stream_done();
       if (a.finish)
         hipLaunchKernelGGL((slice_finish_kernel<3>), dim3((unsigned)((a.npos + 255) / 256)), dim3(256), 0, s, net,
-                           a.part, a.pinfo, (uint64_t)a.npos, (uint32_t)n, a.out_parent, a.out_child);
+                           a.part, a.pinfo, (uint64_t)a.npos, (uint32_t)n, a.out_parent, a.out_child, packed);
     } else {
       hipLaunchKernelGGL((stream_eval_kernel<3072>), dim3(g), dim3(384), 0, s, net, a.offsets, (uint32_t)n, K, B0, B1,
                          a.swz, a.eoff, a.ent, a.tiles, a.btiles, a.order, a.out_parent, a.out_child, a.pool, scr, a.err,
-                         a.pool + 64, 0, nullptr, (uint64_t)0, nullptr);
+                         a.pool + 64, 0, nullptr, (uint64_t)0, nullptr, 0);
       stream_done();
     }
   } else if (net.L1 == 1024) {
@@ -1315,7 +1328,7 @@
     if (do_stream) {
       hipLaunchKernelGGL((stream_eval_kernel<1024>), dim3(g), dim3(128), 0, s, net, a.offsets, (uint32_t)n, K, B0, B1,
                          a.swz, a.eoff, a.ent, a.tiles, a.btiles, a.order, a.out_parent, a.out_child, a.pool, scr, a.err,
-                         a.pool + 64, 0, nullptr, (uint64_t)0, nullptr);
+                         a.pool + 64, 0, nullptr, (uint64_t)0, nullptr, 0);
       stream_done();
     }
   } else {
diff --git a/fishnet_amd/gpu_nnue.py b/fishnet_amd/gpu_nnue.py
--- a/fishnet_amd/gpu_nnue.py
+++ b/fishnet_amd/gpu_nnue.py
@@ -42,6 +42,7 @@
 STAT_PLAN_NS, STAT_STREAM_NS, STAT_SCRATCH_PADS, STAT_FINISH_NS = 101, 102, 103, 104
 STAT_BATCH_LAUNCHES, STAT_BATCH_CALLS, STAT_FAST_BATCHES, STAT_FAST_FALLBACKS = 117, 118, 119, 120
 STAT_RANK_NS = 121
+STAT_PART_BYTES = 122
 HOST_STAGES = {"parse": 110, "upload": 111, "replay": 112, "compute": 113, "download": 114, "tail": 115, "total": 116}
 EXPAND_STAGES = ["count_scan", "total_readback", "write_children", "classify", "small_net", "big_net", "finalize",
                  "score"]
diff --git a/include/gpu_nnue.h b/include/gpu_nnue.h
--- a/include/gpu_nnue.h
+++ b/include/gpu_nnue.h
@@ -53,6 +53,7 @@
 #define GN_STAT_HOST_TAIL_NS 115
 #define GN_STAT_HOST_TOTAL_NS 116
 #define GN_STAT_RANK_NS 121
+#define GN_STAT_PART_BYTES 122
 #define GN_STAT_BATCH_LAUNCHES 117
 #define GN_STAT_BATCH_CALLS 118
 #define GN_STAT_FAST_BATCHES 119
diff --git a/rust/gpu-nnue-sys/src/lib.rs b/rust/gpu-nnue-sys/src/lib.rs
--- a/rust/gpu-nnue-sys/src/lib.rs
+++ b/rust/gpu-nnue-sys/src/lib.rs
@@ -44,6 +44,7 @@
 pub const GN_STAT_FAST_BATCHES: c_int = 119;
 pub const GN_STAT_FAST_FALLBACKS: c_int = 120;
 pub const GN_STAT_RANK_NS: c_int = 121;
+pub const GN_STAT_PART_BYTES: c_int = 122;
 
 pub const GN_FLAG_IN_CHECK: u16 = 1;
 pub const GN_FLAG_SMALLNET: u16 = 2;
```

Result: no change. 860.2 million (median of 6 runs) (+0.9%).
